# jhbastek/PhysicsInformedDiffusionModels

Hardware: NVIDIA H100
Metric: train samples/s Darcy 64x64 PIDM (higher is better)
Workload: dtype bf16

## Files before the change

### include/pidm.h

```cpp
#ifndef PIDM_H_
#define PIDM_H_

#ifdef __cplusplus
extern "C" {
#endif

#ifndef PIDM_F32
#define PIDM_F32 0
#define PIDM_BF16 1
#endif

const char* pidm_last_error(void);
int pidm_version(void);

int pidm_qsample(const float* x0, const float* noise, const long long* t, const float* sqrt_ab,
                 const float* sqrt_1mab, float* xt, int B, int per_sample, void* stream);
int pidm_posterior_step(const float* x_t, const float* x0_pred, const float* z, float* out, float coef1, float coef2,
                        float sigma, long long n, void* stream);
int pidm_axpby_per_sample(const float* a, const float* x, const float* b, const float* y, const float* c,
                          const float* z, float* out, int B, int per_sample, void* stream);
int pidm_ddim_coefs(const long long* t, const long long* t_next, const float* posterior_mean_coef1,
                    const float* posterior_mean_coef2, const float* sqrt_recip_alphas, const float* noise_mean_coeff,
                    const float* alphas_prod, float* coef_x0, float* coef_x, int B, void* stream);
int pidm_scale(const float* x, const float* alpha_dev, float* out, long long n, void* stream);

int pidm_toy_pidm_loss(const float* target, const float* output, const float* residual, const float* ineq,
                       const float* opt, const long long* t, const float* p2_loss_weight,
                       const float* posterior_var_clipped, float c_data, float c_residual, float c_ineq, float lambda_opt,
                       float* sums7, float* grad_output, float* grad_residual, float* grad_ineq, float* grad_opt, int B,
                       int D, void* stream);

#define PIDM_DARCY_PIXELS_AT_BOUNDARY 1
#define PIDM_DARCY_PERIODIC 2
int pidm_darcy_residual_fwd(const float* x0hat, const float* f_s, float* residual, int B, int pixels,
                            float domain_length, int reverse_d1, int flags, void* stream);
int pidm_darcy_residual_bwd(const float* x0hat, const float* f_s, const float* grad_residual, float* grad_x0hat, int B,
                            int pixels, float domain_length, int reverse_d1, int flags, void* stream);
#define PIDM_FD_PERIODIC 8
int pidm_fd_stencil(const float* u, float* out, int planes, int pixels, int mode, float d0, float d1, void* stream);
int pidm_darcy_pidm_loss(const float* x0hat, const float* model_out, const float* target, const float* f_s,
                         const long long* t, const float* p2_loss_weight, const float* posterior_var_clipped,
                         float c_data, float c_residual, float* sums3, float* grad_x0hat, float* grad_model_out, int B,
                         int pixels, float domain_length, int reverse_d1, int flags, void* stream);
int pidm_darcy_jacobian_max(const float* x0hat, float* max_dr_dp, int B, int pixels, float domain_length, int reverse_d1,
                            int flags, void* stream);

int pidm_nchw_to_nhwc(const float* src, void* dst, int B, int C, int HW, int Cpad, int dtype, void* stream);
int pidm_nhwc_to_nchw(const void* src, float* dst, int B, int C, int HW, int Cpad, int dtype, void* stream);
int pidm_add(const void* a, const void* b, void* out, long long n, int dtype, void* stream);
int pidm_gelu_fwd(const void* x, void* y, long long n, int dtype, void* stream);
int pidm_gelu_bwd(const void* x, const void* dy, void* dx, long long n, int dtype, void* stream);
int pidm_concat_channels(const void* a, const void* b, void* out, long long rows, int Ca, int Cb, int dtype, void* stream);
int pidm_split_channels(const void* g, void* ga, void* gb, long long rows, int Ca, int Cb, int dtype, void* stream);

int pidm_pack_entry_size(void);
int pidm_pack_weights(const void* table_dev, int n_entries, int dtype, void* stream);
int pidm_pack_pair_entry_size(void);
int pidm_pack_weights_pairs(const void* table_dev, const int* tile_map_dev, int tile_base, int n_tiles, int max_taps,
                            int dtype, void* stream);
int pidm_conv2d_simt(const void* x, const void* w_packed, const float* bias, const void* residual, void* y, int B,
                     int H, int W, int Cin, int Ho, int Wo, int Cout, int KH, int KW, int stride, int pad,
                     int transposed, int dtype, void* stream);
int pidm_conv2d_wgrad_simt(const void* x, const void* dy, float* dw, float* dbias, int B, int H, int W, int Cin,
                           int Cin_real, int Ho, int Wo, int Cout, int KH, int KW, int stride, int pad, int transposed,
                           long long w_stride_n, long long w_stride_c, int dtype, void* stream);
int pidm_debug_set_trace(void* buf);
int pidm_conv2d_tc_general(const void* x, const void* w_packed, const float* bias, const void* residual, void* y, int B,
                           int H, int W, int Cin, int Ho, int Wo, int Cout, int KH, int KW, int stride, int pad,
                           int transposed, float* gn_sums, int gn_groups, int gn_sums_zeroed, void* stream);
int pidm_conv2d_tc_general_supported(int B, int H, int W, int Cin, int Ho, int Wo, int Cout, int KH, int KW, int stride,
                                     int pad, int transposed);
int pidm_conv2d_tc_plan(int B, int H, int W, int Cin, int Ho, int Wo, int Cout, int KH, int KW, int stride, int pad,
                        int transposed, int* out);
int pidm_conv2d_wgrad_tc(const void* a, const void* b, float* dw, int B, int HA, int WA, int CA, int CA_real, int GH,
                         int GW, int CB, int KH, int KW, int a_stride, int pad, long long s_row, long long s_col,
                         void* stream);
int pidm_conv2d_wgrad_tc_supported(int B, int GH, int GW, int CA, int CB, int KH, int KW, int a_stride);
int pidm_conv2d_wgrad_tc_plan(int B, int HA, int WA, int CA, int CA_real, int GH, int GW, int CB, int KH, int KW,
                              int a_stride, int pad, long long s_row, long long s_col, int* out);
int pidm_colsum(const void* x, float* out, long long M, int C, int dtype, void* stream);

int pidm_groupnorm_silu_fwd(const void* x, const float* gamma, const float* beta, const float* scale_shift,
                            const void* residual, void* y, float* sums, int stats_precomputed, int B, int HW, int C, int G,
                            float eps, int dtype, void* stream);
int pidm_groupnorm_silu_bwd(const void* x, const void* dy, const float* sums, const float* gamma, const float* beta,
                            const float* scale_shift, void* dx, float* dgamma, float* dbeta, float* d_scale_shift,
                            float* dbias_of_producer, float* workspace, int B, int HW, int C, int G, float eps,
                            int dtype, void* stream);
int pidm_layernorm_c_fwd(const void* x, const float* gamma, void* y, long long M, int C, float eps, int dtype, void* stream);
int pidm_layernorm_c_bwd(const void* x, const void* dy, const float* gamma, void* dx, float* dgamma,
                         const void* dx_residual , long long M, int C,
                         float eps, int dtype, void* stream);

int pidm_linattn_fused_supported(int C, int heads, int N, int dtype);
int pidm_linattn_fused_workspace_floats(int B, int N);
int pidm_linattn_fused_plan(int B, int N, int* out);
int pidm_linattn_fused_fwd(const void* xn, const void* w_qkv, void* out, float* ctx, float* kmax, float* kzinv,
                           float* workspace, int B, int N, void* stream);
int pidm_linattn_fused_bwd(const void* xn, const void* w_qkv, const void* dout, const float* ctx, const float* kmax,
                           const float* kzinv, void* dxn, float* dctx, int B, int N, void* stream);
int pidm_linattn_fused_wgrad(const void* xn, const void* w_qkv, const void* dout, const float* ctx, const float* dctx,
                             const float* kmax, const float* kzinv, float* grad_w, int B, int N, long long w_stride_n,
                             long long w_stride_c, void* stream);
int pidm_linattn_workspace_floats(int B, int N, int heads);
int pidm_linattn_fwd(const void* qkv, void* out, float* ctx, float* kmax, float* kzinv, float* workspace, int B, int N,
                     int heads, int dtype, void* stream);
int pidm_linattn_bwd(const void* qkv, const void* dout, const float* ctx, const float* kmax, const float* kzinv,
                     void* dqkv, float* dctx_scratch, int B, int N, int heads, int dtype, void* stream);
int pidm_attn_fwd(const void* qkv, void* out, int B, int n_tokens, int heads, int dtype, void* stream);
int pidm_attn_bwd(const void* qkv, const void* dout, void* dqkv, int B, int n_tokens, int heads, int dtype, void* stream);

int pidm_time_embed_fwd(const long long* t, const float* W1, const float* b1, const float* W2, const float* b2,
                        float* emb, float* h1, float* temb, float* silu_t, int B, int dim, int td, void* stream);
int pidm_time_embed_bwd(const float* d_silu_t, const float* emb, const float* h1, const float* temb, const float* W2,
                        float* dW1, float* db1, float* dW2, float* db2, float* workspace, int B, int dim, int td,
                        int parts, void* stream);
int pidm_mlp_entry_size(void);
int pidm_block_mlps_fwd(const void* table_dev, int n_entries, int max_rows, const float* silu_t, int B, int td,
                        void* stream);
int pidm_block_mlps_bwd(const void* table_dev, int n_entries, int max_rows, const float* silu_t, float* d_silu_t, int B,
                        int td, int parts, void* stream);

int pidm_head_fwd(const void* x, const float* w, const float* bias, float* y, int B, int HW, int C, int O,
                  int sigmoid_last, int dtype, void* stream);
int pidm_head_bwd(const void* x, const float* w, const float* y, const float* dy, void* dx, float* dw, float* db, int B,
                  int HW, int C, int O, int sigmoid_last, int dtype, void* stream);

int pidm_sumsq(const float* x, long long n, float* out, float* workspace, void* stream);
int pidm_adam_ema_step(float* param, float* grad, float* exp_avg, float* exp_avg_sq, float* ema_shadow, long long n,
                       float lr, double beta1, double beta2, float eps, int step, int* step_counter_dev,
                       const float* grad_norm_sq_dev, float grad_scale, float max_norm, float ema_mu,
                       int ema_first_step, int zero_grad, void* stream);

int pidm_mechanics_residual_fwd(const float* u, const float* rho, const float* bcs, const float* KE, float* residual,
                                float* compliance, int B, int nel, void* stream);
int pidm_mechanics_residual_bwd(const float* u, const float* rho, const float* bcs, const float* KE,
                                const float* grad_residual, const float* grad_compliance, float* grad_u, float* grad_rho,
                                float* workspace , int B, int nel, void* stream);
int pidm_mech_pidm_loss(const float* u, const float* rho, const float* x0, const float* residual, const float* compliance,
                        const float* vf, const long long* t, const float* p2_loss_weight,
                        const float* posterior_var_clipped, float c_data, float c_residual, float c_ineq,
                        float lambda_opt, float* sums6, float* grad_u, float* grad_rho, float* grad_residual,
                        float* grad_compliance, int B, int nel, void* stream);
int pidm_bilinear_resize_fwd(const float* x, float* y, int planes, int in, int out, void* stream);
int pidm_bilinear_resize_bwd(const float* dy, float* dx, int planes, int in, int out, void* stream);

#ifdef __cplusplus
}
#endif
#endif
```

### physicsinformeddiffusionmodels_b200/_lib.py

```python
import ctypes
import os

import torch

_HERE = os.path.dirname(os.path.abspath(__file__))
LIB_PATH = os.path.join(_HERE, 'libpidm.so')

P = ctypes.c_void_p
I = ctypes.c_int
L = ctypes.c_longlong
F = ctypes.c_float
D = ctypes.c_double

_SIGS = {
    'pidm_qsample': [P, P, P, P, P, P, I, I, P],
    'pidm_posterior_step': [P, P, P, P, F, F, F, L, P],
    'pidm_scale': [P, P, P, L, P],
    'pidm_ddim_coefs': [P, P, P, P, P, P, P, P, P, I, P],
    'pidm_axpby_per_sample': [P, P, P, P, P, P, P, I, I, P],
    'pidm_toy_pidm_loss': [P, P, P, P, P, P, P, P, F, F, F, F, P, P, P, P, P, I, I, P],
    'pidm_fd_stencil': [P, P, I, I, I, F, F, P],
    'pidm_darcy_residual_fwd': [P, P, P, I, I, F, I, I, P],
    'pidm_darcy_residual_bwd': [P, P, P, P, I, I, F, I, I, P],
    'pidm_darcy_jacobian_max': [P, P, I, I, F, I, I, P],
    'pidm_darcy_pidm_loss': [P, P, P, P, P, P, P, F, F, P, P, P, I, I, F, I, I, P],
    'pidm_nchw_to_nhwc': [P, P, I, I, I, I, I, P],
    'pidm_nhwc_to_nchw': [P, P, I, I, I, I, I, P],
    'pidm_add': [P, P, P, L, I, P],
    'pidm_gelu_fwd': [P, P, L, I, P],
    'pidm_gelu_bwd': [P, P, P, L, I, P],
    'pidm_concat_channels': [P, P, P, L, I, I, I, P],
    'pidm_split_channels': [P, P, P, L, I, I, I, P],
    'pidm_pack_entry_size': [],
    'pidm_pack_weights': [P, I, I, P],
    'pidm_pack_pair_entry_size': [],
    'pidm_pack_weights_pairs': [P, P, I, I, I, I, P],
    'pidm_conv2d_simt': [P, P, P, P, P, I, I, I, I, I, I, I, I, I, I, I, I, I, P],
    'pidm_conv2d_wgrad_simt': [P, P, P, P, I, I, I, I, I, I, I, I, I, I, I, I, I, L, L, I, P],
    'pidm_debug_set_trace': [P],
    'pidm_conv2d_tc_general': [P, P, P, P, P, I, I, I, I, I, I, I, I, I, I, I, I, P, I, I, P],
    'pidm_conv2d_tc_general_supported': [I, I, I, I, I, I, I, I, I, I, I, I],
    'pidm_conv2d_tc_plan': [I, I, I, I, I, I, I, I, I, I, I, I, P],
    'pidm_conv2d_wgrad_tc': [P, P, P, I, I, I, I, I, I, I, I, I, I, I, I, L, L, P],
    'pidm_conv2d_wgrad_tc_supported': [I, I, I, I, I, I, I, I],
    'pidm_conv2d_wgrad_tc_plan': [I, I, I, I, I, I, I, I, I, I, I, I, L, L, P],
    'pidm_colsum': [P, P, L, I, I, P],
    'pidm_groupnorm_silu_fwd': [P, P, P, P, P, P, P, I, I, I, I, I, F, I, P],
    'pidm_groupnorm_silu_bwd': [P, P, P, P, P, P, P, P, P, P, P, P, I, I, I, I, F, I, P],
    'pidm_layernorm_c_fwd': [P, P, P, L, I, F, I, P],
    'pidm_layernorm_c_bwd': [P, P, P, P, P, P, L, I, F, I, P],
    'pidm_linattn_workspace_floats': [I, I, I],
    'pidm_linattn_fused_supported': [I, I, I, I],
    'pidm_linattn_fused_workspace_floats': [I, I],
    'pidm_linattn_fused_plan': [I, I, P],
    'pidm_linattn_fused_fwd': [P, P, P, P, P, P, P, I, I, P],
    'pidm_linattn_fused_bwd': [P, P, P, P, P, P, P, P, I, I, P],
    'pidm_linattn_fused_wgrad': [P, P, P, P, P, P, P, P, I, I, L, L, P],
    'pidm_linattn_fwd': [P, P, P, P, P, P, I, I, I, I, P],
    'pidm_linattn_bwd': [P, P, P, P, P, P, P, I, I, I, I, P],
    'pidm_attn_fwd': [P, P, I, I, I, I, P],
    'pidm_attn_bwd': [P, P, P, I, I, I, I, P],
    'pidm_time_embed_fwd': [P, P, P, P, P, P, P, P, P, I, I, I, P],
    'pidm_time_embed_bwd': [P, P, P, P, P, P, P, P, P, P, I, I, I, I, P],
    'pidm_mlp_entry_size': [],
    'pidm_block_mlps_fwd': [P, I, I, P, I, I, P],
    'pidm_block_mlps_bwd': [P, I, I, P, P, I, I, I, P],
    'pidm_head_fwd': [P, P, P, P, I, I, I, I, I, I, P],
    'pidm_head_bwd': [P, P, P, P, P, P, P, I, I, I, I, I, I, P],
    'pidm_sumsq': [P, L, P, P, P],
    'pidm_adam_ema_step': [P, P, P, P, P, L, F, D, D, F, I, P, P, F, F, F, I, I, P],
    'pidm_mechanics_residual_fwd': [P, P, P, P, P, P, I, I, P],
    'pidm_mechanics_residual_bwd': [P, P, P, P, P, P, P, P, P, I, I, P],
    'pidm_mech_pidm_loss': [P, P, P, P, P, P, P, P, P, F, F, F, F, P, P, P, P, P, I, I, P],
    'pidm_bilinear_resize_fwd': [P, P, I, I, I, P],
    'pidm_bilinear_resize_bwd': [P, P, I, I, I, P],
    'pidm_version': [],
}
_VALUE_RETURN = {'pidm_pack_entry_size', 'pidm_pack_pair_entry_size', 'pidm_mlp_entry_size', 'pidm_linattn_workspace_floats', 'pidm_version',
                 'pidm_linattn_fused_supported', 'pidm_linattn_fused_workspace_floats',
                 'pidm_conv2d_tc_supported', 'pidm_conv2d_wgrad_tc_supported', 'pidm_conv2d_tc_general_supported',
                 'pidm_conv2d_tc_plan', 'pidm_conv2d_wgrad_tc_plan', 'pidm_linattn_fused_plan'}

if not os.path.exists(LIB_PATH):
    raise ImportError(f'{LIB_PATH} is missing: build it with `python __graft_entry__.py` (nvcc, sm_90a). '
                      'There is no CPU / PyTorch fallback for the PIDM hot path.')

_lib = ctypes.CDLL(LIB_PATH)
_lib.pidm_last_error.restype = ctypes.c_char_p
_lib.pidm_last_error.argtypes = []
for _n, _a in _SIGS.items():
    _f = getattr(_lib, _n)
    _f.argtypes = _a
    _f.restype = ctypes.c_int

launch_count = 0


def exported_symbols():
    return sorted(_SIGS) + ['pidm_last_error']


def ptr(t):
    if t is None:
        return None
    return t.data_ptr()


def stream():
    return torch.cuda.current_stream().cuda_stream


def call(name, *args):
    global launch_count
    conv = []
    for a in args:
        if isinstance(a, torch.Tensor):
            conv.append(a.data_ptr())
        else:
            conv.append(a)
    rc = getattr(_lib, name)(*conv)
    if name in _VALUE_RETURN:
        return rc
    launch_count += 1
    if rc != 0:
        raise RuntimeError(f'{name} failed (code {rc}): {_lib.pidm_last_error().decode()}')
    return 0


DTYPE_CODE = {torch.float32: 0, torch.bfloat16: 1}
```

### physicsinformeddiffusionmodels_b200/csrc/attention_fused.cu

```cuda
#define PIDM_PDL_GROUP 1
#include "common.cuh"
#include "mma_util.cuh"
#include "pidm.h"

namespace pidm {

constexpr int LF_C = 32;

__device__ __forceinline__ uint32_t movm_t(uint32_t x) {
    uint32_t y;
    asm volatile("movmatrix.sync.aligned.m8n8.trans.b16 %0, %1;" : "=r"(y) : "r"(x));
    return y;
}

__device__ __forceinline__ void load_w_frags(uint32_t (&w)[2][4][2], const __nv_bfloat16* __restrict__ Wrows, int lane) {
    const int g = lane >> 2, t = lane & 3;
#pragma unroll
    for (int ks = 0; ks < 2; ++ks)
#pragma unroll
        for (int nt = 0; nt < 4; ++nt) {
            const uint32_t* row = reinterpret_cast<const uint32_t*>(Wrows + (size_t)(nt * 8 + g) * LF_C + ks * 16 + 2 * t);
            w[ks][nt][0] = __ldg(row);
            w[ks][nt][1] = __ldg(row + 4);
        }
}
template <int MT>
__device__ __forceinline__ void load_x_frags(uint32_t (&a)[MT][2][4], const __nv_bfloat16* Xs, int lane) {
#pragma unroll
    for (int mt = 0; mt < MT; ++mt)
#pragma unroll
        for (int ks = 0; ks < 2; ++ks) frag_a_rowmajor(a[mt][ks], Xs, LW_PITCH, mt * 16, ks * 16, lane);
}
template <int MT>
__device__ __forceinline__ void project(float (&c)[MT][4][4], const uint32_t (&a)[MT][2][4], const uint32_t (&w)[2][4][2]) {
#pragma unroll
    for (int mt = 0; mt < MT; ++mt)
#pragma unroll
        for (int nt = 0; nt < 4; ++nt) {
#pragma unroll
            for (int i = 0; i < 4; ++i) c[mt][nt][i] = 0.f;
#pragma unroll
            for (int ks = 0; ks < 2; ++ks) mma_bf16(c[mt][nt], a[mt][ks], w[ks][nt][0], w[ks][nt][1]);
        }
}
__device__ __forceinline__ void frag_softmax(float (&c)[4][4], float mul) {
#pragma unroll
    for (int half = 0; half < 2; ++half) {
        float mx = -INFINITY;
#pragma unroll
        for (int nt = 0; nt < 4; ++nt) mx = fmaxf(mx, fmaxf(c[nt][half * 2], c[nt][half * 2 + 1]));
        mx = fmaxf(mx, __shfl_xor_sync(0xffffffffu, mx, 1));
        mx = fmaxf(mx, __shfl_xor_sync(0xffffffffu, mx, 2));
        float s = 0.f;
#pragma unroll
        for (int nt = 0; nt < 4; ++nt) {
            c[nt][half * 2] = __expf(c[nt][half * 2] - mx);
            c[nt][half * 2 + 1] = __expf(c[nt][half * 2 + 1] - mx);
            s += c[nt][half * 2] + c[nt][half * 2 + 1];
        }
        s += __shfl_xor_sync(0xffffffffu, s, 1);
        s += __shfl_xor_sync(0xffffffffu, s, 2);
        const float inv = mul / s;
#pragma unroll
        for (int nt = 0; nt < 4; ++nt) { c[nt][half * 2] *= inv; c[nt][half * 2 + 1] *= inv; }
    }
}
__device__ __forceinline__ void c_to_a(uint32_t (&a)[2][4], const float (&c)[4][4]) {
#pragma unroll
    for (int ks = 0; ks < 2; ++ks) {
        a[ks][0] = pack_bf16(c[2 * ks][0], c[2 * ks][1]);
        a[ks][1] = pack_bf16(c[2 * ks][2], c[2 * ks][3]);
        a[ks][2] = pack_bf16(c[2 * ks + 1][0], c[2 * ks + 1][1]);
        a[ks][3] = pack_bf16(c[2 * ks + 1][2], c[2 * ks + 1][3]);
    }
}
__device__ __forceinline__ void load_cols(float (&v)[8], const float* __restrict__ src, int lane) {
    const int t = lane & 3;
#pragma unroll
    for (int nt = 0; nt < 4; ++nt) { v[nt * 2] = src[nt * 8 + 2 * t]; v[nt * 2 + 1] = src[nt * 8 + 2 * t + 1]; }
}

constexpr int LFS_STAGES = 2;
__global__ void __launch_bounds__(256) laf_kmax_kernel(const __nv_bfloat16* __restrict__ xn,
                                                       const __nv_bfloat16* __restrict__ W, float* __restrict__ part,
                                                       int N, int rows_per_chunk) {
    pdl_trigger();
    pdl_wait();
    extern __shared__ __align__(16) unsigned char raw[];
    const int b = blockIdx.y, chunk = blockIdx.x, lane = threadIdx.x & 31, h = threadIdx.x >> 5;
    __nv_bfloat16* ring = reinterpret_cast<__nv_bfloat16*>(raw) + (size_t)h * (LFS_STAGES * LW_TILE);
    const int n_begin = chunk * rows_per_chunk, n_end = min(N, n_begin + rows_per_chunk);
    const int n_tiles = (n_end - n_begin) / 32;
    const __nv_bfloat16* xsrc = xn + ((size_t)b * N + n_begin) * LF_C;
    auto issue = [&](int it) {
        if (it < n_tiles) lw_issue<32>(ring + (size_t)(it % LFS_STAGES) * LW_TILE, xsrc + (size_t)it * 32 * LF_C, LF_C, lane);
        cp_commit();
    };
#pragma unroll
    for (int s = 0; s < LFS_STAGES; ++s) issue(s);
    uint32_t wk[2][4][2];
    load_w_frags(wk, W + (size_t)(LM_HID + h * LM_D) * LF_C, lane);
    float m[8];
#pragma unroll
    for (int i = 0; i < 8; ++i) m[i] = -INFINITY;
    for (int it = 0; it < n_tiles; ++it) {
        cp_wait<LFS_STAGES - 1>();
        __syncwarp();
        uint32_t ax[2][2][4];
        load_x_frags<2>(ax, ring + (size_t)(it % LFS_STAGES) * LW_TILE, lane);
        __syncwarp();
        issue(it + LFS_STAGES);
        float ck[2][4][4];
        project<2>(ck, ax, wk);
#pragma unroll
        for (int nt = 0; nt < 4; ++nt)
#pragma unroll
            for (int j = 0; j < 2; ++j)
                m[nt * 2 + j] = fmaxf(fmaxf(m[nt * 2 + j], fmaxf(ck[0][nt][j], ck[0][nt][2 + j])),
                                      fmaxf(ck[1][nt][j], ck[1][nt][2 + j]));
    }
#pragma unroll
    for (int off = 4; off < 32; off <<= 1)
#pragma unroll
        for (int i = 0; i < 8; ++i) m[i] = fmaxf(m[i], __shfl_xor_sync(0xffffffffu, m[i], off));
    if (lane < 4) {
        float* o = part + ((size_t)b * gridDim.x + chunk) * LM_HID + h * LM_D;
#pragma unroll
        for (int nt = 0; nt < 4; ++nt)
#pragma unroll
            for (int j = 0; j < 2; ++j) o[nt * 8 + 2 * lane + j] = m[nt * 2 + j];
    }
}

__global__ void laf_finalize_kernel(float* __restrict__ ctx, float* __restrict__ kzinv, int n_rows) {
    pdl_trigger();
    pdl_wait();
    const int row = blockIdx.x * (blockDim.x / 32) + (threadIdx.x >> 5), lane = threadIdx.x & 31;
    if (row >= n_rows) return;
    const float zi = 1.f / kzinv[row];
    ctx[(size_t)row * LM_D + lane] *= zi;
    __syncwarp();
    if (lane == 0) kzinv[row] = zi;
}

template <int MODE>
struct LfcCfg {
    static constexpr int STAGES = MODE == 0 ? 4 : 2;
    static constexpr int STAGE_ELEMS = MODE == 0 ? LW_TILE : 2 * LW_TILE;
    static constexpr size_t SMEM = (size_t)LM_HEADS * STAGES * STAGE_ELEMS * 2 + (size_t)LM_HEADS * 2 * LM_D * 4;
};
template <int MODE>
__global__ void __launch_bounds__(256, 2) laf_ctx_kernel(const __nv_bfloat16* __restrict__ xn, const __nv_bfloat16* __restrict__ W,
                                                      const __nv_bfloat16* __restrict__ dout, const float* __restrict__ part,
                                                      int n_stat_chunks, float* __restrict__ kmax, float* __restrict__ kzinv,
                                                      float* __restrict__ ctx, int N, int chunk_px, float scale) {
    pdl_trigger();
    pdl_wait();
    extern __shared__ __align__(16) unsigned char raw[];
    constexpr int LFC_STAGES = LfcCfg<MODE>::STAGES, LFC_STAGE_ELEMS = LfcCfg<MODE>::STAGE_ELEMS;
    const int b = blockIdx.y, chunk = blockIdx.x, lane = threadIdx.x & 31, h = threadIdx.x >> 5;
    __nv_bfloat16* ring = reinterpret_cast<__nv_bfloat16*>(raw) + (size_t)h * (LFC_STAGES * LFC_STAGE_ELEMS);
    float* sM = reinterpret_cast<float*>(raw + (size_t)LM_HEADS * LFC_STAGES * LFC_STAGE_ELEMS * 2) + h * 2 * LM_D;
    float* sZi = sM + LM_D;
    const int n_begin = chunk * chunk_px, n_end = min(N, n_begin + chunk_px);
    const int n_tiles = (n_end - n_begin) / 32;
    const size_t pix0 = (size_t)b * N + n_begin;
    const __nv_bfloat16* xsrc = xn + pix0 * LF_C;
    const __nv_bfloat16* gsrc = (MODE == 1) ? dout + pix0 * LM_HID + h * LM_D : nullptr;
    auto issue = [&](int it) {
        if (it < n_tiles) {
            __nv_bfloat16* buf = ring + (size_t)(it % LFC_STAGES) * LFC_STAGE_ELEMS;
            lw_issue<32>(buf, xsrc + (size_t)it * 32 * LF_C, LF_C, lane);
            if (MODE == 1) lw_issue<32>(buf + LW_TILE, gsrc + (size_t)it * 32 * LM_HID, LM_HID, lane);
        }
        cp_commit();
    };
#pragma unroll
    for (int s = 0; s < LFC_STAGES; ++s) issue(s);
    uint32_t w0[2][4][2], w1[2][4][2];
    load_w_frags(w0, W + (size_t)((MODE == 0 ? LM_HID : 0) + h * LM_D) * LF_C, lane);
    if (MODE == 0) load_w_frags(w1, W + (size_t)(2 * LM_HID + h * LM_D) * LF_C, lane);
    float Mc[8];
    float zacc[8];
#pragma unroll
    for (int i = 0; i < 8; ++i) zacc[i] = 0.f;
    if (MODE == 0) {
        const int c = h * LM_D + lane;
        float M = -INFINITY;
        for (int i = 0; i < n_stat_chunks; ++i) M = fmaxf(M, part[((size_t)b * n_stat_chunks + i) * LM_HID + c]);
        sM[lane] = M;
        if (chunk == 0) kmax[(size_t)b * LM_HID + c] = M;
        __syncwarp();
        load_cols(Mc, sM, lane);
    }
    float acc[2][4][4];
#pragma unroll
    for (int i = 0; i < 2; ++i)
#pragma unroll
        for (int j = 0; j < 4; ++j)
#pragma unroll
            for (int k = 0; k < 4; ++k) acc[i][j][k] = 0.f;
    for (int it = 0; it < n_tiles; ++it) {
        cp_wait<LFC_STAGES - 1>();
        __syncwarp();
        const __nv_bfloat16* buf = ring + (size_t)(it % LFC_STAGES) * LFC_STAGE_ELEMS;
        uint32_t ax[2][2][4];
        load_x_frags<2>(ax, buf, lane);
        uint32_t bv[2][4][2];
        if (MODE == 1) {
#pragma unroll
            for (int ks = 0; ks < 2; ++ks) {
                uint32_t b01[4], b23[4];
                frag_b_krows(b01, buf + LW_TILE, LW_PITCH, ks * 16, 0, lane);
                frag_b_krows(b23, buf + LW_TILE, LW_PITCH, ks * 16, 16, lane);
                bv[ks][0][0] = b01[0]; bv[ks][0][1] = b01[1]; bv[ks][1][0] = b01[2]; bv[ks][1][1] = b01[3];
                bv[ks][2][0] = b23[0]; bv[ks][2][1] = b23[1]; bv[ks][3][0] = b23[2]; bv[ks][3][1] = b23[3];
            }
        }
        __syncwarp();
        issue(it + LFC_STAGES);
        float cw[2][4][4];
        project<2>(cw, ax, w0);
        if (MODE == 0) {
#pragma unroll
            for (int mt = 0; mt < 2; ++mt)
#pragma unroll
                for (int nt = 0; nt < 4; ++nt)
#pragma unroll
                    for (int i = 0; i < 4; ++i) {
                        cw[mt][nt][i] = __expf(cw[mt][nt][i] - Mc[nt * 2 + (i & 1)]);
                        zacc[nt * 2 + (i & 1)] += cw[mt][nt][i];
                    }
            float cv[2][4][4];
            project<2>(cv, ax, w1);
#pragma unroll
            for (int mt = 0; mt < 2; ++mt)
#pragma unroll
                for (int nt = 0; nt < 4; ++nt) {
                    bv[mt][nt][0] = movm_t(pack_bf16(cv[mt][nt][0], cv[mt][nt][1]));
                    bv[mt][nt][1] = movm_t(pack_bf16(cv[mt][nt][2], cv[mt][nt][3]));
                }
        } else {
            frag_softmax(cw[0], scale);
            frag_softmax(cw[1], scale);
        }
#pragma unroll
        for (int mt = 0; mt < 2; ++mt) {
#pragma unroll
            for (int md = 0; md < 2; ++md) {
                uint32_t a[4];
                a[0] = movm_t(pack_bf16(cw[mt][2 * md][0], cw[mt][2 * md][1]));
                a[1] = movm_t(pack_bf16(cw[mt][2 * md + 1][0], cw[mt][2 * md + 1][1]));
                a[2] = movm_t(pack_bf16(cw[mt][2 * md][2], cw[mt][2 * md][3]));
                a[3] = movm_t(pack_bf16(cw[mt][2 * md + 1][2], cw[mt][2 * md + 1][3]));
#pragma unroll
                for (int ne = 0; ne < 4; ++ne) mma_bf16(acc[md][ne], a, bv[mt][ne][0], bv[mt][ne][1]);
            }
        }
    }
    const int g = lane >> 2, t = lane & 3;
    if (MODE == 0) {
#pragma unroll
        for (int off = 4; off < 32; off <<= 1)
#pragma unroll
            for (int i = 0; i < 8; ++i) zacc[i] += __shfl_xor_sync(0xffffffffu, zacc[i], off);
        if (lane < 4) {
#pragma unroll
            for (int nt = 0; nt < 4; ++nt)
#pragma unroll
                for (int j = 0; j < 2; ++j)
                    atomicAdd(kzinv + (size_t)b * LM_HID + h * LM_D + nt * 8 + 2 * lane + j, zacc[nt * 2 + j]);
        }
    }
    float* cb = ctx + ((size_t)b * LM_HEADS + h) * LM_D * LM_D;
#pragma unroll
    for (int md = 0; md < 2; ++md)
#pragma unroll
        for (int half = 0; half < 2; ++half) {
            const int d = md * 16 + g + half * 8;
            const float f = (MODE == 0) ? 1.f / (float)N : 1.f;
#pragma unroll
            for (int ne = 0; ne < 4; ++ne) {
                const int e = ne * 8 + 2 * t;
                atomicAdd(cb + d * LM_D + e, acc[md][ne][half * 2] * f);
                atomicAdd(cb + d * LM_D + e + 1, acc[md][ne][half * 2 + 1] * f);
            }
        }
}

constexpr int LFO_STAGES = 2;
__global__ void __launch_bounds__(256) laf_out_kernel(const __nv_bfloat16* __restrict__ xn, const __nv_bfloat16* __restrict__ W,
                                                      const float* __restrict__ ctx, __nv_bfloat16* __restrict__ out, int N,
                                                      int chunk_px, float scale) {
    pdl_trigger();
    pdl_wait();
    extern __shared__ __align__(16) unsigned char raw[];
    const int b = blockIdx.y, chunk = blockIdx.x, lane = threadIdx.x & 31, h = threadIdx.x >> 5;
    __nv_bfloat16* ring = reinterpret_cast<__nv_bfloat16*>(raw) + (size_t)h * ((LFO_STAGES + 1) * LW_TILE);
    __nv_bfloat16* Os = ring + LFO_STAGES * LW_TILE;
    const int n_begin = chunk * chunk_px, n_end = min(N, n_begin + chunk_px);
    const int n_tiles = (n_end - n_begin) / 32;
    const size_t pix0 = (size_t)b * N + n_begin;
    const __nv_bfloat16* xsrc = xn + pix0 * LF_C;
    __nv_bfloat16* odst = out + pix0 * LM_HID + h * LM_D;
    auto issue = [&](int it) {
        if (it < n_tiles) lw_issue<32>(ring + (size_t)(it % LFO_STAGES) * LW_TILE, xsrc + (size_t)it * 32 * LF_C, LF_C, lane);
        cp_commit();
    };
#pragma unroll
    for (int s = 0; s < LFO_STAGES; ++s) issue(s);
    uint32_t wq[2][4][2];
    load_w_frags(wq, W + (size_t)(h * LM_D) * LF_C, lane);
    const float* ch = ctx + ((size_t)b * LM_HEADS + h) * LM_D * LM_D;
    uint32_t bf[2][4][2];
#pragma unroll
    for (int ks = 0; ks < 2; ++ks)
#pragma unroll
        for (int nt = 0; nt < 4; ++nt) frag_b_global<true>(bf[ks][nt], ch, ks * 16, nt * 8, lane);
    const int g = lane >> 2, t = lane & 3;
    for (int it = 0; it < n_tiles; ++it) {
        cp_wait<LFO_STAGES - 1>();
        __syncwarp();
        uint32_t ax[2][2][4];
        load_x_frags<2>(ax, ring + (size_t)(it % LFO_STAGES) * LW_TILE, lane);
        __syncwarp();
        issue(it + LFO_STAGES);
        float cq[2][4][4];
        project<2>(cq, ax, wq);
#pragma unroll
        for (int mt = 0; mt < 2; ++mt) {
            frag_softmax(cq[mt], scale);
            uint32_t a[2][4];
            c_to_a(a, cq[mt]);
            float c[4][4];
#pragma unroll
            for (int i = 0; i < 4; ++i)
#pragma unroll
                for (int k = 0; k < 4; ++k) c[i][k] = 0.f;
#pragma unroll
            for (int ks = 0; ks < 2; ++ks)
#pragma unroll
                for (int nt = 0; nt < 4; ++nt) mma_bf16(c[nt], a[ks], bf[ks][nt][0], bf[ks][nt][1]);
#pragma unroll
            for (int nt = 0; nt < 4; ++nt) {
                __nv_bfloat16* o = Os + (size_t)(mt * 16 + g) * LW_PITCH + nt * 8 + 2 * t;
                *reinterpret_cast<uint32_t*>(o) = pack_bf16(c[nt][0], c[nt][1]);
                *reinterpret_cast<uint32_t*>(o + 8 * LW_PITCH) = pack_bf16(c[nt][2], c[nt][3]);
            }
        }
        __syncwarp();
        lw_store<32>(odst + (size_t)it * 32 * LM_HID, LM_HID, Os, lane);
        __syncwarp();
    }
}

constexpr int LFB_ROWS = 16;
constexpr int LFB_STAGES = 4;
constexpr int LFB_TILE = LFB_ROWS * LW_PITCH;

struct LfbTile {
    uint32_t ax[1][2][4], ag[2][4];
};
__device__ __forceinline__ void lfb_dq(float (&dq)[4][4], const LfbTile& tl, const uint32_t (&wq)[2][4][2],
                                       const uint32_t (&bc)[2][4][2], float scale) {
    float c1[1][4][4], c2[4][4];
    project<1>(c1, tl.ax, wq);
    frag_softmax(c1[0], 1.f);
#pragma unroll
    for (int nt = 0; nt < 4; ++nt) {
#pragma unroll
        for (int i = 0; i < 4; ++i) c2[nt][i] = 0.f;
#pragma unroll
        for (int ks = 0; ks < 2; ++ks) mma_bf16(c2[nt], tl.ag[ks], bc[ks][nt][0], bc[ks][nt][1]);
    }
#pragma unroll
    for (int half = 0; half < 2; ++half) {
        float dot = 0.f;
#pragma unroll
        for (int nt = 0; nt < 4; ++nt)
            dot += c1[0][nt][half * 2] * c2[nt][half * 2] + c1[0][nt][half * 2 + 1] * c2[nt][half * 2 + 1];
        dot += __shfl_xor_sync(0xffffffffu, dot, 1);
        dot += __shfl_xor_sync(0xffffffffu, dot, 2);
#pragma unroll
        for (int nt = 0; nt < 4; ++nt)
#pragma unroll
            for (int j = 0; j < 2; ++j) dq[nt][half * 2 + j] = scale * c1[0][nt][half * 2 + j] * (c2[nt][half * 2 + j] - dot);
    }
}
__device__ __forceinline__ void lfb_dkdv(float (&dk)[4][4], float (&dv)[4][4], const uint32_t (&ax)[1][2][4],
                                         const uint32_t (&wk)[2][4][2], const uint32_t (&wv)[2][4][2],
                                         const uint32_t (&bd)[2][4][2], const uint32_t (&bt)[2][4][2],
                                         const float (&Mc)[8], const float (&Zc)[8], const float (&cdc)[8], float invN) {
    float c1[1][4][4];
    uint32_t a[2][4];
    project<1>(c1, ax, wv);
    c_to_a(a, c1[0]);
#pragma unroll
    for (int nt = 0; nt < 4; ++nt) {
#pragma unroll
        for (int i = 0; i < 4; ++i) dk[nt][i] = 0.f;
#pragma unroll
        for (int ks = 0; ks < 2; ++ks) mma_bf16(dk[nt], a[ks], bd[ks][nt][0], bd[ks][nt][1]);
    }
    project<1>(c1, ax, wk);
#pragma unroll
    for (int nt = 0; nt < 4; ++nt)
#pragma unroll
        for (int i = 0; i < 4; ++i) {
            c1[0][nt][i] = __expf(c1[0][nt][i] - Mc[nt * 2 + (i & 1)]) * Zc[nt * 2 + (i & 1)];
            dk[nt][i] = c1[0][nt][i] * (dk[nt][i] * invN - cdc[nt * 2 + (i & 1)]);
        }
    c_to_a(a, c1[0]);
#pragma unroll
    for (int nt = 0; nt < 4; ++nt) {
#pragma unroll
        for (int i = 0; i < 4; ++i) dv[nt][i] = 0.f;
#pragma unroll
        for (int ks = 0; ks < 2; ++ks) mma_bf16(dv[nt], a[ks], bt[ks][nt][0], bt[ks][nt][1]);
#pragma unroll
        for (int i = 0; i < 4; ++i) dv[nt][i] *= invN;
    }
}
__device__ __forceinline__ void lfb_cd(float (&cdc)[8], float* scd, const float* __restrict__ cg, const float* __restrict__ dg,
                                       int lane) {
    float s = 0.f;
#pragma unroll
    for (int e = 0; e < LM_D; e += 4) {
        const float4 x = *reinterpret_cast<const float4*>(dg + lane * LM_D + e);
        const float4 y = *reinterpret_cast<const float4*>(cg + lane * LM_D + e);
        s += x.x * y.x + x.y * y.y + x.z * y.z + x.w * y.w;
    }
    scd[lane] = s;
    __syncwarp();
    load_cols(cdc, scd, lane);
}

constexpr int LFB_STAGE_ELEMS = (1 + LM_HEADS) * LFB_TILE;
constexpr int LFB_W_PITCH = LF_C + 8;
constexpr int LFB_R_PITCH = LF_C + 8;
constexpr size_t LAF_BWD_SMEM = (size_t)LFB_STAGES * LFB_STAGE_ELEMS * 2 + (size_t)3 * LM_HID * LFB_W_PITCH * 2 +
                                (size_t)LM_HEADS * LFB_ROWS * LFB_R_PITCH * 4 + (size_t)LM_HEADS * LM_D * 4;

__device__ __forceinline__ void mma_w(float (&c)[4][4], const uint32_t (&g)[2][4], const __nv_bfloat16* Wh, int lane) {
#pragma unroll
    for (int kd = 0; kd < 2; ++kd)
#pragma unroll
        for (int np = 0; np < 2; ++np) {
            uint32_t bw[4];
            frag_b_krows(bw, Wh, LFB_W_PITCH, kd * 16, np * 16, lane);
            mma_bf16(c[2 * np], g[kd], bw[0], bw[1]);
            mma_bf16(c[2 * np + 1], g[kd], bw[2], bw[3]);
        }
}

__global__ void __launch_bounds__(256) laf_bwd_kernel(const __nv_bfloat16* __restrict__ xn, const __nv_bfloat16* __restrict__ W,
                                                      const __nv_bfloat16* __restrict__ dout, const float* __restrict__ ctx,
                                                      const float* __restrict__ dctx, const float* __restrict__ kmax,
                                                      const float* __restrict__ kzinv, __nv_bfloat16* __restrict__ dxn,
                                                      int N, int chunk_px, float scale) {
    pdl_trigger();
    pdl_wait();
    extern __shared__ __align__(16) unsigned char raw[];
    const int b = blockIdx.y, chunk = blockIdx.x, lane = threadIdx.x & 31, h = threadIdx.x >> 5;
    __nv_bfloat16* ring = reinterpret_cast<__nv_bfloat16*>(raw);
    __nv_bfloat16* Ws = ring + LFB_STAGES * LFB_STAGE_ELEMS;
    float* R = reinterpret_cast<float*>(Ws + 3 * LM_HID * LFB_W_PITCH);
    float* scd = R + LM_HEADS * LFB_ROWS * LFB_R_PITCH + h * LM_D;
    const int n_begin = chunk * chunk_px, n_end = min(N, n_begin + chunk_px);
    const int n_tiles = (n_end - n_begin) / LFB_ROWS;
    const size_t pix0 = (size_t)b * N + n_begin;
    const __nv_bfloat16* xsrc = xn + pix0 * LF_C;
    const __nv_bfloat16* gsrc = dout + pix0 * LM_HID + h * LM_D;
    for (int i = threadIdx.x; i < 3 * LM_HID * (LF_C / 8); i += blockDim.x)
        cp_async16(Ws + (i >> 2) * LFB_W_PITCH + (i & 3) * 8, W + (size_t)(i >> 2) * LF_C + (i & 3) * 8);
    cp_commit();
    auto issue = [&](int it) {
        if (it < n_tiles) {
            __nv_bfloat16* buf = ring + (size_t)(it % LFB_STAGES) * LFB_STAGE_ELEMS;
            if (h == 0) lw_issue<LFB_ROWS>(buf, xsrc + (size_t)it * LFB_ROWS * LF_C, LF_C, lane);
            lw_issue<LFB_ROWS>(buf + (1 + h) * LFB_TILE, gsrc + (size_t)it * LFB_ROWS * LM_HID, LM_HID, lane);
        }
        cp_commit();
    };
#pragma unroll
    for (int s = 0; s < LFB_STAGES - 1; ++s) issue(s);
    const float* cg = ctx + ((size_t)b * LM_HEADS + h) * LM_D * LM_D;
    const float* dg = dctx + ((size_t)b * LM_HEADS + h) * LM_D * LM_D;
    float Mc[8], Zc[8], cdc[8];
    lfb_cd(cdc, scd, cg, dg, lane);
    load_cols(Mc, kmax + (size_t)b * LM_HID + h * LM_D, lane);
    load_cols(Zc, kzinv + (size_t)b * LM_HID + h * LM_D, lane);
    uint32_t wq[2][4][2], wk[2][4][2], wv[2][4][2];
    load_w_frags(wq, W + (size_t)(h * LM_D) * LF_C, lane);
    load_w_frags(wk, W + (size_t)(LM_HID + h * LM_D) * LF_C, lane);
    load_w_frags(wv, W + (size_t)(2 * LM_HID + h * LM_D) * LF_C, lane);
    uint32_t bc[2][4][2], bd[2][4][2], bt[2][4][2];
#pragma unroll
    for (int ks = 0; ks < 2; ++ks)
#pragma unroll
        for (int nt = 0; nt < 4; ++nt) {
            frag_b_global<false>(bc[ks][nt], cg, ks * 16, nt * 8, lane);
            frag_b_global<false>(bd[ks][nt], dg, ks * 16, nt * 8, lane);
            frag_b_global<true>(bt[ks][nt], dg, ks * 16, nt * 8, lane);
        }
    const int g = lane >> 2, t = lane & 3;
    const float invN = 1.f / (float)N;
    const __nv_bfloat16* Wq = Ws + (size_t)(h * LM_D) * LFB_W_PITCH;
    const __nv_bfloat16* Wk = Wq + (size_t)LM_HID * LFB_W_PITCH;
    const __nv_bfloat16* Wv = Wk + (size_t)LM_HID * LFB_W_PITCH;
    float* Rw = R + h * LFB_ROWS * LFB_R_PITCH;
    const int rrow = threadIdx.x >> 4, rcol = (threadIdx.x & 15) * 2;
    for (int it = 0; it < n_tiles; ++it) {
        cp_wait<LFB_STAGES - 2>();
        __syncthreads();
        issue(it + LFB_STAGES - 1);
        const __nv_bfloat16* buf = ring + (size_t)(it % LFB_STAGES) * LFB_STAGE_ELEMS;
        LfbTile tl;
        load_x_frags<1>(tl.ax, buf, lane);
        frag_a_rowmajor(tl.ag[0], buf + (1 + h) * LFB_TILE, LW_PITCH, 0, 0, lane);
        frag_a_rowmajor(tl.ag[1], buf + (1 + h) * LFB_TILE, LW_PITCH, 0, 16, lane);
        float dx[4][4];
#pragma unroll
        for (int nt = 0; nt < 4; ++nt)
#pragma unroll
            for (int i = 0; i < 4; ++i) dx[nt][i] = 0.f;
        uint32_t a[2][4];
        {
            float dq[4][4];
            lfb_dq(dq, tl, wq, bc, scale);
            c_to_a(a, dq);
            mma_w(dx, a, Wq, lane);
        }
        {
            float dk[4][4], dv[4][4];
            lfb_dkdv(dk, dv, tl.ax, wk, wv, bd, bt, Mc, Zc, cdc, invN);
            c_to_a(a, dk);
            mma_w(dx, a, Wk, lane);
            c_to_a(a, dv);
            mma_w(dx, a, Wv, lane);
        }
#pragma unroll
        for (int nt = 0; nt < 4; ++nt)
#pragma unroll
            for (int half = 0; half < 2; ++half)
                *reinterpret_cast<float2*>(Rw + (g + half * 8) * LFB_R_PITCH + nt * 8 + 2 * t) =
                    make_float2(dx[nt][half * 2], dx[nt][half * 2 + 1]);
        __syncthreads();
        float sx = 0.f, sy = 0.f;
#pragma unroll
        for (int w = 0; w < LM_HEADS; ++w) {
            const float2 v = *reinterpret_cast<const float2*>(R + (w * LFB_ROWS + rrow) * LFB_R_PITCH + rcol);
            sx += v.x;
            sy += v.y;
        }
        *reinterpret_cast<uint32_t*>(dxn + (pix0 + (size_t)it * LFB_ROWS + rrow) * LF_C + rcol) = pack_bf16(sx, sy);
    }
}

template <int PART>
struct LfwCfg {
    static constexpr int MATS = PART == 0 ? 1 : 2;
    static constexpr int STAGE_ELEMS = (PART == 0 ? 2 : 1) * LFB_TILE;
    static constexpr int S_PITCH = LM_D + 1;
    static_assert(LFB_STAGES * STAGE_ELEMS * 2 >= LM_D * S_PITCH * 4, "the epilogue staging reuses the tile ring");
    static constexpr size_t SMEM = (size_t)LM_HEADS * (LFB_STAGES * STAGE_ELEMS * 2 + LM_D * 4);
};

__device__ __forceinline__ void acc_gtx(float (&acc)[2][4][4], const float (&gf)[4][4], const uint32_t (&bx)[2][4]) {
#pragma unroll
    for (int md = 0; md < 2; ++md) {
        uint32_t a[4];
        a[0] = movm_t(pack_bf16(gf[2 * md][0], gf[2 * md][1]));
        a[1] = movm_t(pack_bf16(gf[2 * md + 1][0], gf[2 * md + 1][1]));
        a[2] = movm_t(pack_bf16(gf[2 * md][2], gf[2 * md][3]));
        a[3] = movm_t(pack_bf16(gf[2 * md + 1][2], gf[2 * md + 1][3]));
#pragma unroll
        for (int np = 0; np < 2; ++np) {
            mma_bf16(acc[md][2 * np], a, bx[np][0], bx[np][1]);
            mma_bf16(acc[md][2 * np + 1], a, bx[np][2], bx[np][3]);
        }
    }
}

template <int PART>
__global__ void __launch_bounds__(256) laf_wgrad_kernel(const __nv_bfloat16* __restrict__ xn, const __nv_bfloat16* __restrict__ W,
                                                        const __nv_bfloat16* __restrict__ dout, const float* __restrict__ ctx,
                                                        const float* __restrict__ dctx, const float* __restrict__ kmax,
                                                        const float* __restrict__ kzinv, float* __restrict__ grad_w, int N,
                                                        int chunk_px, long long w_stride_n, long long w_stride_c, float scale) {
    pdl_trigger();
    pdl_wait();
    extern __shared__ __align__(16) unsigned char raw[];
    constexpr int MATS = LfwCfg<PART>::MATS, STAGE_ELEMS = LfwCfg<PART>::STAGE_ELEMS, S_PITCH = LfwCfg<PART>::S_PITCH;
    const int b = blockIdx.y, chunk = blockIdx.x, lane = threadIdx.x & 31, h = threadIdx.x >> 5;
    __nv_bfloat16* ring = reinterpret_cast<__nv_bfloat16*>(raw) + (size_t)h * (LFB_STAGES * STAGE_ELEMS);
    float* scd = reinterpret_cast<float*>(raw + (size_t)LM_HEADS * LFB_STAGES * STAGE_ELEMS * 2) + h * LM_D;
    const int n_begin = chunk * chunk_px, n_end = min(N, n_begin + chunk_px);
    const int n_tiles = (n_end - n_begin) / LFB_ROWS;
    const size_t pix0 = (size_t)b * N + n_begin;
    const __nv_bfloat16* xsrc = xn + pix0 * LF_C;
    const __nv_bfloat16* gsrc = dout + pix0 * LM_HID + h * LM_D;
    auto issue = [&](int it) {
        if (it < n_tiles) {
            __nv_bfloat16* buf = ring + (size_t)(it % LFB_STAGES) * STAGE_ELEMS;
            lw_issue<LFB_ROWS>(buf, xsrc + (size_t)it * LFB_ROWS * LF_C, LF_C, lane);
            if (PART == 0) lw_issue<LFB_ROWS>(buf + LFB_TILE, gsrc + (size_t)it * LFB_ROWS * LM_HID, LM_HID, lane);
        }
        cp_commit();
    };
#pragma unroll
    for (int s = 0; s < LFB_STAGES; ++s) issue(s);
    const float* cg = ctx + ((size_t)b * LM_HEADS + h) * LM_D * LM_D;
    const float* dg = dctx + ((size_t)b * LM_HEADS + h) * LM_D * LM_D;
    float Mc[8], Zc[8], cdc[8];
    uint32_t w0[2][4][2], w1[2][4][2];
    uint32_t b0[2][4][2], b1[2][4][2];
    if (PART == 0) {
        load_w_frags(w0, W + (size_t)(h * LM_D) * LF_C, lane);
    } else {
        lfb_cd(cdc, scd, cg, dg, lane);
        load_cols(Mc, kmax + (size_t)b * LM_HID + h * LM_D, lane);
        load_cols(Zc, kzinv + (size_t)b * LM_HID + h * LM_D, lane);
        load_w_frags(w0, W + (size_t)(LM_HID + h * LM_D) * LF_C, lane);
        load_w_frags(w1, W + (size_t)(2 * LM_HID + h * LM_D) * LF_C, lane);
    }
#pragma unroll
    for (int ks = 0; ks < 2; ++ks)
#pragma unroll
        for (int nt = 0; nt < 4; ++nt) {
            frag_b_global<false>(b0[ks][nt], PART == 0 ? cg : dg, ks * 16, nt * 8, lane);
            if (PART == 1) frag_b_global<true>(b1[ks][nt], dg, ks * 16, nt * 8, lane);
        }
    const float invN = 1.f / (float)N;
    float acc[MATS][2][4][4];
#pragma unroll
    for (int m = 0; m < MATS; ++m)
#pragma unroll
        for (int i = 0; i < 2; ++i)
#pragma unroll
            for (int j = 0; j < 4; ++j)
#pragma unroll
                for (int k = 0; k < 4; ++k) acc[m][i][j][k] = 0.f;
    for (int it = 0; it < n_tiles; ++it) {
        cp_wait<LFB_STAGES - 1>();
        __syncwarp();
        const __nv_bfloat16* buf = ring + (size_t)(it % LFB_STAGES) * STAGE_ELEMS;
        LfbTile tl;
        load_x_frags<1>(tl.ax, buf, lane);
        uint32_t bx[2][4];
        frag_b_krows(bx[0], buf, LW_PITCH, 0, 0, lane);
        frag_b_krows(bx[1], buf, LW_PITCH, 0, 16, lane);
        if (PART == 0) {
            frag_a_rowmajor(tl.ag[0], buf + LFB_TILE, LW_PITCH, 0, 0, lane);
            frag_a_rowmajor(tl.ag[1], buf + LFB_TILE, LW_PITCH, 0, 16, lane);
        }
        __syncwarp();
        issue(it + LFB_STAGES);
        if (PART == 0) {
            float dq[4][4];
            lfb_dq(dq, tl, w0, b0, scale);
            acc_gtx(acc[0], dq, bx);
        } else {
            float dk[4][4], dv[4][4];
            lfb_dkdv(dk, dv, tl.ax, w0, w1, b0, b1, Mc, Zc, cdc, invN);
            acc_gtx(acc[0], dk, bx);
            acc_gtx(acc[MATS - 1], dv, bx);
        }
    }
    cp_wait<0>();
    __syncwarp();
    float* S = reinterpret_cast<float*>(ring);
    const int g = lane >> 2, t = lane & 3;
#pragma unroll
    for (int m = 0; m < MATS; ++m) {
#pragma unroll
        for (int md = 0; md < 2; ++md)
#pragma unroll
            for (int nc = 0; nc < 4; ++nc)
#pragma unroll
                for (int i = 0; i < 4; ++i) S[(md * 16 + g + 8 * (i >> 1)) * S_PITCH + nc * 8 + 2 * t + (i & 1)] = acc[m][md][nc][i];
        __syncwarp();
        float* dst = grad_w + (long long)((PART + m) * LM_HID + h * LM_D) * w_stride_n + lane * w_stride_c;
#pragma unroll 4
        for (int d = 0; d < LM_D; ++d) atomicAdd(dst + d * w_stride_n, S[d * S_PITCH + lane]);
        __syncwarp();
    }
}

constexpr size_t LAF_STATS_SMEM = (size_t)LM_HEADS * LFS_STAGES * LW_TILE * 2;
constexpr size_t LAF_OUT_SMEM = (size_t)LM_HEADS * (LFO_STAGES + 1) * LW_TILE * 2;

static int laf_attrs() {
    static bool done = false;
    if (!done) {
        PIDM_CUDA(cudaFuncSetAttribute(laf_kmax_kernel, cudaFuncAttributeMaxDynamicSharedMemorySize, (int)LAF_STATS_SMEM));
        PIDM_CUDA(cudaFuncSetAttribute(laf_ctx_kernel<0>, cudaFuncAttributeMaxDynamicSharedMemorySize, (int)LfcCfg<0>::SMEM));
        PIDM_CUDA(cudaFuncSetAttribute(laf_ctx_kernel<1>, cudaFuncAttributeMaxDynamicSharedMemorySize, (int)LfcCfg<1>::SMEM));
        PIDM_CUDA(cudaFuncSetAttribute(laf_out_kernel, cudaFuncAttributeMaxDynamicSharedMemorySize, (int)LAF_OUT_SMEM));
        PIDM_CUDA(cudaFuncSetAttribute(laf_bwd_kernel, cudaFuncAttributeMaxDynamicSharedMemorySize, (int)LAF_BWD_SMEM));
        PIDM_CUDA(cudaFuncSetAttribute(laf_wgrad_kernel<0>, cudaFuncAttributeMaxDynamicSharedMemorySize, (int)LfwCfg<0>::SMEM));
        PIDM_CUDA(cudaFuncSetAttribute(laf_wgrad_kernel<1>, cudaFuncAttributeMaxDynamicSharedMemorySize, (int)LfwCfg<1>::SMEM));
        done = true;
    }
    return 0;
}

static int laf_chunk_px(int B, int N, int ctas_per_sm) {
    int k = (num_sms() * ctas_per_sm) / B;
    if (k < 1) k = 1;
    int px = ((N + k - 1) / k + 31) / 32 * 32;
    if (px < 64) px = 64;
    if (px > N) px = N;
    return px;
}
static int laf_stat_chunks(int N) {
    int c = N / 128;
    if (c < 1) c = 1;
    if (c > 16) c = 16;
    return c;
}

}
using namespace pidm;

extern "C" int pidm_linattn_fused_supported(int C, int heads, int N, int dtype) {
    return (C == LF_C && heads == LM_HEADS && dtype == PIDM_BF16 && N % 128 == 0) ? 1 : 0;
}

extern "C" int pidm_linattn_fused_workspace_floats(int B, int N) { return B * laf_stat_chunks(N) * LM_HID; }

extern "C" int pidm_linattn_fused_plan(int B, int N, int* out) {
    PIDM_REQUIRE(N % 128 == 0 && B > 0, "linattn_fused_plan: N must be a multiple of 128 (got %d)", N);
    const int v[5] = {laf_stat_chunks(N), laf_chunk_px(B, N, 2), laf_chunk_px(B, N, 3), laf_chunk_px(B, N, 1),
                      laf_chunk_px(B, N, 1)};
    for (int i = 0; i < 5; ++i) out[i] = v[i];
    return 0;
}

extern "C" int pidm_linattn_fused_fwd(const void* xn, const void* w_qkv, void* out, float* ctx, float* kmax, float* kzinv,
                                      float* workspace, int B, int N, void* stream) {
    PIDM_REQUIRE(N % 128 == 0, "linattn_fused: N must be a multiple of 128 (got %d)", N);
    cudaStream_t st = (cudaStream_t)stream;
    if (int e = laf_attrs()) return e;
    const float scale = 0.17677669529663687f;
    const __nv_bfloat16* x = (const __nv_bfloat16*)xn;
    const __nv_bfloat16* w = (const __nv_bfloat16*)w_qkv;
    PIDM_CUDA(cudaMemsetAsync(ctx, 0, (size_t)B * LM_HEADS * LM_D * LM_D * sizeof(float), st));
    PIDM_CUDA(cudaMemsetAsync(kzinv, 0, (size_t)B * LM_HID * sizeof(float), st));
    const int chunks = laf_stat_chunks(N);
    const int rpc = N / chunks;
    PIDM_REQUIRE(rpc % 32 == 0 && rpc * chunks == N, "linattn_fused: bad statistics chunking for N=%d", N);
    PIDM_CUDA(launch_pdl(laf_kmax_kernel, dim3(dim3(chunks, B)), dim3(256), (size_t)(LAF_STATS_SMEM), st, x, w, workspace, N, rpc));
    const int cpx = laf_chunk_px(B, N, 2);
    PIDM_CUDA(launch_pdl(laf_ctx_kernel<0>, dim3(dim3((N + cpx - 1) / cpx, B)), dim3(256), (size_t)(LfcCfg<0>::SMEM), st, x, w, nullptr, workspace, chunks, kmax, kzinv,
                                                                             ctx, N, cpx, scale));
    PIDM_CUDA(launch_pdl(laf_finalize_kernel, dim3((B * LM_HID + 7) / 8), dim3(256), (size_t)(0), st, ctx, kzinv, B * LM_HID));
    const int opx = laf_chunk_px(B, N, 3);
    PIDM_CUDA(launch_pdl(laf_out_kernel, dim3(dim3((N + opx - 1) / opx, B)), dim3(256), (size_t)(LAF_OUT_SMEM), st, x, w, ctx, (__nv_bfloat16*)out, N, opx, scale));
    PIDM_LAUNCH_CHECK("linattn_fused_fwd");
    return 0;
}

extern "C" int pidm_linattn_fused_bwd(const void* xn, const void* w_qkv, const void* dout, const float* ctx,
                                      const float* kmax, const float* kzinv, void* dxn, float* dctx, int B, int N,
                                      void* stream) {
    PIDM_REQUIRE(N % 128 == 0, "linattn_fused: N must be a multiple of 128 (got %d)", N);
    cudaStream_t st = (cudaStream_t)stream;
    if (int e = laf_attrs()) return e;
    const float scale = 0.17677669529663687f;
    const __nv_bfloat16* x = (const __nv_bfloat16*)xn;
    const __nv_bfloat16* w = (const __nv_bfloat16*)w_qkv;
    PIDM_CUDA(cudaMemsetAsync(dctx, 0, (size_t)B * LM_HEADS * LM_D * LM_D * sizeof(float), st));
    const int cpx = laf_chunk_px(B, N, 2);
    PIDM_CUDA(launch_pdl(laf_ctx_kernel<1>, dim3(dim3((N + cpx - 1) / cpx, B)), dim3(256), (size_t)(LfcCfg<1>::SMEM), st, x, w, (const __nv_bfloat16*)dout, nullptr, 0,
                                                                             nullptr, nullptr, dctx, N, cpx, scale));
    const int bpx = laf_chunk_px(B, N, 1);
    PIDM_CUDA(launch_pdl(laf_bwd_kernel, dim3(dim3((N + bpx - 1) / bpx, B)), dim3(256), (size_t)(LAF_BWD_SMEM), st, x, w, (const __nv_bfloat16*)dout, ctx, dctx, kmax,
                                                                          kzinv, (__nv_bfloat16*)dxn, N, bpx, scale));
    PIDM_LAUNCH_CHECK("linattn_fused_bwd");
    return 0;
}

extern "C" int pidm_linattn_fused_wgrad(const void* xn, const void* w_qkv, const void* dout, const float* ctx,
                                        const float* dctx, const float* kmax, const float* kzinv, float* grad_w, int B,
                                        int N, long long w_stride_n, long long w_stride_c, void* stream) {
    PIDM_REQUIRE(N % 128 == 0, "linattn_fused: N must be a multiple of 128 (got %d)", N);
    cudaStream_t st = (cudaStream_t)stream;
    if (int e = laf_attrs()) return e;
    const float scale = 0.17677669529663687f;
    const __nv_bfloat16* x = (const __nv_bfloat16*)xn;
    const __nv_bfloat16* w = (const __nv_bfloat16*)w_qkv;
    const __nv_bfloat16* g = (const __nv_bfloat16*)dout;
    const int px = laf_chunk_px(B, N, 1);
    const dim3 grid((N + px - 1) / px, B);
    PIDM_CUDA(launch_pdl(laf_wgrad_kernel<0>, grid, dim3(256), LfwCfg<0>::SMEM, st, x, w, g, ctx, dctx, kmax, kzinv, grad_w, N,
                         px, w_stride_n, w_stride_c, scale));
    PIDM_CUDA(launch_pdl(laf_wgrad_kernel<1>, grid, dim3(256), LfwCfg<1>::SMEM, st, x, w, g, ctx, dctx, kmax, kzinv, grad_w, N,
                         px, w_stride_n, w_stride_c, scale));
    PIDM_LAUNCH_CHECK("linattn_fused_wgrad");
    return 0;
}
```

### physicsinformeddiffusionmodels_b200/ops.py

```python
import os

import torch

from . import _lib
from ._lib import call, stream

_TC_HARD_OFF = os.environ.get('PIDM_DISABLE_TC') == '1'
_STATE = {'act_dtype': torch.bfloat16, 'use_tc': not _TC_HARD_OFF}


def set_precision(name):
    _STATE['act_dtype'] = {'bf16': torch.bfloat16, 'fp32': torch.float32}[name]


def set_tensor_core_conv(flag):
    _STATE['use_tc'] = bool(flag) and not _TC_HARD_OFF


def act_dtype():
    return _STATE['act_dtype']


def _code(t):
    return _lib.DTYPE_CODE[t.dtype]


def _grad_buffer(p):
    g = getattr(p, '_pidm_grad', None)
    if g is not None:
        return g, None
    z = torch.zeros_like(p)
    return z, z


def _need_cuda(*ts):
    for t in ts:
        if t is not None and not t.is_cuda:
            raise RuntimeError('physicsinformeddiffusionmodels_b200 runs on CUDA (H100) only: got a CPU tensor. '
                               'There is no CPU fallback on the product path.')


def _need_f32(**named):
    for k, t in named.items():
        if t is None:
            continue
        if not t.is_cuda:
            raise RuntimeError(f'{k}: expected a CUDA tensor (no CPU fallback on the product path)')
        if t.dtype != torch.float32 or not t.is_contiguous():
            raise RuntimeError(f'{k}: expected a contiguous float32 tensor, got {t.dtype}, strides {t.stride()}')


def nchw_to_nhwc(x, cpad, dtype=None):
    _need_cuda(x)
    B, C, H, W = x.shape
    dtype = dtype or act_dtype()
    y = torch.empty(B, H, W, cpad, device=x.device, dtype=dtype)
    call('pidm_nchw_to_nhwc', x.contiguous().float(), y, B, C, H * W, cpad, _lib.DTYPE_CODE[dtype], stream())
    return y


def nhwc_to_nchw(x, C=None):
    B, H, W, Cp = x.shape
    C = C or Cp
    y = torch.empty(B, C, H, W, device=x.device, dtype=torch.float32)
    call('pidm_nhwc_to_nchw', x, y, B, C, H * W, Cp, _code(x), stream())
    return y


class _Add(torch.autograd.Function):
    @staticmethod
    def forward(ctx, a, b):
        o = torch.empty_like(a)
        call('pidm_add', a, b, o, a.numel(), _code(a), stream())
        return o

    @staticmethod
    def backward(ctx, g):
        return g, g


def add(a, b):
    return _Add.apply(a.contiguous(), b.contiguous())


class _Gelu(torch.autograd.Function):
    @staticmethod
    def forward(ctx, x):
        y = torch.empty_like(x)
        call('pidm_gelu_fwd', x, y, x.numel(), _code(x), stream())
        ctx.save_for_backward(x)
        return y

    @staticmethod
    def backward(ctx, dy):
        (x,) = ctx.saved_tensors
        dx = torch.empty_like(x)
        call('pidm_gelu_bwd', x, dy.contiguous(), dx, x.numel(), _code(x), stream())
        return dx


def gelu(x):
    return _Gelu.apply(x.contiguous())


class _Stash(torch.autograd.Function):

    @staticmethod
    def forward(ctx, x, link):
        ctx.link = link
        link['expect_skip'] = True
        return x.view_as(x)

    @staticmethod
    def backward(ctx, g):
        ctx.link['skip'] = g.contiguous()
        return None, None


def stash_grad(x, link):
    return _Stash.apply(x, link)


def _take_skip(link):
    if link is None or not link.get('expect_skip'):
        return None
    if 'skip' not in link:
        raise RuntimeError('skip-connection gradient was expected but has not been produced yet (autograd order)')
    return link.pop('skip')


class _Concat(torch.autograd.Function):
    @staticmethod
    def forward(ctx, a, b):
        B, H, W, Ca = a.shape
        Cb = b.shape[-1]
        o = torch.empty(B, H, W, Ca + Cb, device=a.device, dtype=a.dtype)
        call('pidm_concat_channels', a, b, o, B * H * W, Ca, Cb, _code(a), stream())
        ctx.shapes = (a.shape, b.shape)
        return o

    @staticmethod
    def backward(ctx, g):
        sa, sb = ctx.shapes
        g = g.contiguous()
        ga = torch.empty(sa, device=g.device, dtype=g.dtype)
        gb = torch.empty(sb, device=g.device, dtype=g.dtype)
        call('pidm_split_channels', g, ga, gb, sa[0] * sa[1] * sa[2], sa[3], sb[3], _code(g), stream())
        return ga, gb


def concat(a, b):
    return _Concat.apply(a.contiguous(), b.contiguous())


_ZERO_POOL = {'buf': None, 'cur': 0}


def zero_pool_begin(nfloats, device):
    _ZERO_POOL['buf'] = torch.zeros(int(nfloats), device=device, dtype=torch.float32)
    _ZERO_POOL['cur'] = 0


def zero_pool_end():
    _ZERO_POOL['buf'] = None


def _zero_take(*shape):
    buf = _ZERO_POOL['buf']
    n = 1
    for d in shape:
        n *= int(d)
    n_al = (n + 31) // 32 * 32
    if buf is None or _ZERO_POOL['cur'] + n_al > buf.numel():
        return None
    out = buf[_ZERO_POOL['cur']:_ZERO_POOL['cur'] + n].view(*shape)
    _ZERO_POOL['cur'] += n_al
    return out


def _conv_launch(x, wp, bias, residual, y, g, transposed, gn_sums=None, gn_groups=0, gn_zeroed=False):
    B, H, W, Cin, Ho, Wo, Cout, KH, KW, stride, pad = g
    tr = 1 if transposed else 0
    if (_STATE['use_tc'] and x.dtype == torch.bfloat16
            and call('pidm_conv2d_tc_general_supported', B, H, W, Cin, Ho, Wo, Cout, KH, KW, stride, pad, tr)):
        cpg = Cout // gn_groups if gn_groups else 0
        fuse = gn_sums is not None and (cpg in (4, 8, 16) or (cpg > 0 and cpg % 32 == 0))
        call('pidm_conv2d_tc_general', x, wp, bias, residual, y, B, H, W, Cin, Ho, Wo, Cout, KH, KW, stride, pad, tr,
             gn_sums if fuse else None, gn_groups if fuse else 0, 1 if gn_zeroed else 0, stream())
        return fuse
    else:
        call('pidm_conv2d_simt', x, wp, bias, residual, y, B, H, W, Cin, Ho, Wo, Cout, KH, KW, stride, pad,
             1 if transposed else 0, _code(x), stream())
        return False


class _Conv2d(torch.autograd.Function):

    @staticmethod
    def forward(ctx, x, weight, bias, residual, spec, link, skip):
        B, H, W, Cin = x.shape
        Ho, Wo = spec.out_hw(H, W)
        y = torch.empty(B, Ho, Wo, spec.cout, device=x.device, dtype=x.dtype)
        g = (B, H, W, Cin, Ho, Wo, spec.cout, spec.kh, spec.kw, spec.stride, spec.pad)
        sums, zeroed = None, False
        if link is not None:
            sums = _zero_take(B, link['groups'], 2)
            zeroed = sums is not None
            if sums is None:
                sums = torch.empty(B, link['groups'], 2, device=x.device, dtype=torch.float32)
        fused = _conv_launch(x, spec.wp_fwd, bias, residual, y, g, spec.transposed, sums, link['groups'] if link else 0,
                             zeroed)
        if link is not None:
            link['sums'] = sums if fused else None
            link['bias'] = bias
        ctx.save_for_backward(x, weight, bias)
        ctx.spec, ctx.g, ctx.has_res, ctx.link, ctx.skip = spec, g, residual is not None, link, skip
        if skip is not None and skip[0] == 'park':
            skip[1]['expect_skip'] = True
        return y

    @staticmethod
    def backward(ctx, dy):
        x, weight, bias = ctx.saved_tensors
        dy = dy.contiguous()
        skip = ctx.skip
        dgrad_res = _take_skip(skip[1]) if (skip is not None and skip[0] == 'take' and ctx.needs_input_grad[0]) else None
        dx, gw_ret, gb_ret = _conv_backward(x, weight, bias, ctx.spec, ctx.g, dy, ctx.needs_input_grad[0], ctx.link,
                                            dgrad_res)
        if skip is not None and skip[0] == 'park':
            skip[1]['skip'] = dx
            dx = None
        return dx, gw_ret, gb_ret, (dy if ctx.has_res else None), None, None, None


_SIDE = {'streams': [], 'next': 0, 'keep': [], 'active': False}
_N_SIDE = max(1, int(os.environ.get('PIDM_SIDE_STREAMS', '1')))


def side_stream_begin():
    if os.environ.get('PIDM_NO_SIDE_STREAM') == '1':
        return
    while len(_SIDE['streams']) < _N_SIDE:
        _SIDE['streams'].append(torch.cuda.Stream())
    _SIDE['active'] = True
    _SIDE['next'] = 0
    _SIDE['keep'] = []


def side_stream_join():
    if _SIDE['active']:
        for st in _SIDE['streams']:
            torch.cuda.current_stream().wait_stream(st)
        _SIDE['keep'] = []
        _SIDE['active'] = False


_FORK = {'stream': None}


def fork_stream():
    if _FORK['stream'] is None:
        _FORK['stream'] = torch.cuda.Stream()
    _FORK['stream'].wait_stream(torch.cuda.current_stream())
    return _FORK['stream']


def _wgrad_stream(*operands):
    if not _SIDE['active']:
        return stream()
    side = _SIDE['streams'][_SIDE['next']]
    _SIDE['next'] = (_SIDE['next'] + 1) % len(_SIDE['streams'])
    side.wait_stream(torch.cuda.current_stream())
    _SIDE['keep'].extend(operands)
    return side.cuda_stream


def _conv_backward(x, weight, bias, spec, g, dy, need_dx, link=None, dgrad_residual=None):
    B, H, W, Cin, Ho, Wo, Cout, KH, KW, stride, pad = g
    dx = None
    if need_dx or dgrad_residual is not None:
        dx = torch.empty_like(x)
        if stride == 1 and not spec.transposed:
            gd = (B, Ho, Wo, Cout, H, W, Cin, KH, KW, 1, KH - 1 - pad)
            _conv_launch(dy, spec.wp_dgrad, None, dgrad_residual, dx, gd, False)
        else:
            gd = (B, Ho, Wo, Cout, H, W, Cin, KH, KW, stride, pad)
            _conv_launch(dy, spec.wp_dgrad, None, dgrad_residual, dx, gd, not spec.transposed)
    gw_buf, gw_ret = _grad_buffer(weight)
    gb_buf, gb_ret = (None, None) if bias is None else _grad_buffer(bias)
    if link is not None and 'dbias' in link:
        gb_buf, gb_ret = None, link.pop('dbias')
    use_tc = _STATE['use_tc'] and x.dtype == torch.bfloat16
    ws = _wgrad_stream(x, dy)
    if use_tc and not spec.transposed and call('pidm_conv2d_wgrad_tc_supported', B, Ho, Wo, Cin, Cout, KH, KW, stride):
        call('pidm_conv2d_wgrad_tc', x, dy, gw_buf, B, H, W, Cin, spec.cin_real, Ho, Wo, Cout, KH, KW, stride, pad,
             spec.w_stride_c, spec.w_stride_n, ws)
        if gb_buf is not None:
            call('pidm_colsum', dy, gb_buf, B * Ho * Wo, Cout, _code(dy), ws)
    elif use_tc and spec.transposed and call('pidm_conv2d_wgrad_tc_supported', B, H, W, Cout, Cin, KH, KW, stride):
        call('pidm_conv2d_wgrad_tc', dy, x, gw_buf, B, Ho, Wo, Cout, Cout, H, W, Cin, KH, KW, stride, pad,
             spec.w_stride_n, spec.w_stride_c, ws)
        if gb_buf is not None:
            call('pidm_colsum', dy, gb_buf, B * Ho * Wo, Cout, _code(dy), ws)
    else:
        call('pidm_conv2d_wgrad_simt', x, dy, gw_buf, gb_buf, B, H, W, Cin, spec.cin_real, Ho, Wo, Cout, KH, KW,
             stride, pad, 1 if spec.transposed else 0, spec.w_stride_n, spec.w_stride_c, _code(x), ws)
    return dx, gw_ret, gb_ret


def conv2d(x, weight, bias, spec, residual=None, gn_link=None, skip=None):
    return _Conv2d.apply(x.contiguous(), weight, bias, None if residual is None else residual.contiguous(), spec,
                         gn_link, skip)


class _GroupNormSilu(torch.autograd.Function):
    @staticmethod
    def forward(ctx, x, gamma, beta, scale_shift, groups, eps, link, residual):
        B, H, W, C = x.shape
        y = torch.empty_like(x)
        pre = link is not None and link.get('sums') is not None
        sums = link['sums'] if pre else torch.empty(B, groups, 2, device=x.device, dtype=torch.float32)
        call('pidm_groupnorm_silu_fwd', x, gamma, beta, scale_shift, residual, y, sums, 1 if pre else 0, B, H * W, C,
             groups, eps, _code(x), stream())
        ctx.save_for_backward(x, gamma, beta, scale_shift, sums)
        ctx.groups, ctx.eps, ctx.link, ctx.has_res = groups, eps, link, residual is not None
        return y

    @staticmethod
    def backward(ctx, dy):
        x, gamma, beta, ss, sums = ctx.saved_tensors
        B, H, W, C = x.shape
        dy = dy.contiguous()
        dx = torch.empty_like(x)
        gg_buf, gg_ret = _grad_buffer(gamma)
        gb_buf, gb_ret = _grad_buffer(beta)
        dss = None if ss is None else torch.empty_like(ss)
        ws = torch.empty(B * C * 2, device=x.device, dtype=torch.float32)
        dbias = None
        link = ctx.link
        if link is not None and link.get('bias') is not None:
            dbias, dbias_ret = _grad_buffer(link['bias'])
            link['dbias'] = dbias_ret
        call('pidm_groupnorm_silu_bwd', x, dy, sums, gamma, beta, ss, dx, gg_buf, gb_buf, dss, dbias, ws, B, H * W, C,
             ctx.groups, ctx.eps, _code(x), stream())
        return dx, gg_ret, gb_ret, dss, None, None, None, (dy if ctx.has_res else None)


def groupnorm_silu(x, gamma, beta, scale_shift, groups, eps=1e-5, gn_link=None, residual=None):
    return _GroupNormSilu.apply(x.contiguous(), gamma, beta, scale_shift, groups, eps, gn_link,
                                None if residual is None else residual.contiguous())


class _LayerNormC(torch.autograd.Function):
    @staticmethod
    def forward(ctx, x, gamma, eps, skip_link):
        C = x.shape[-1]
        y = torch.empty_like(x)
        call('pidm_layernorm_c_fwd', x, gamma, y, x.numel() // C, C, eps, _code(x), stream())
        ctx.save_for_backward(x, gamma)
        ctx.eps, ctx.skip_link = eps, skip_link
        return y

    @staticmethod
    def backward(ctx, dy):
        x, gamma = ctx.saved_tensors
        C = x.shape[-1]
        dy = dy.contiguous()
        dx = torch.empty_like(x)
        gg_buf, gg_ret = _grad_buffer(gamma)
        call('pidm_layernorm_c_bwd', x, dy, gamma, dx, gg_buf,
             _take_skip(ctx.skip_link) if ctx.needs_input_grad[0] else None, x.numel() // C, C, ctx.eps,
             _code(x), stream())
        return dx, gg_ret, None, None


def layernorm_c(x, gamma, eps=1e-5, skip_link=None):
    return _LayerNormC.apply(x.contiguous(), gamma, eps, skip_link)


class _LinAttn(torch.autograd.Function):
    @staticmethod
    def forward(ctx, qkv, heads):
        B, H, W, C3 = qkv.shape
        N = H * W
        hid = heads * 32
        assert C3 == 3 * hid
        out = torch.empty(B, H, W, hid, device=qkv.device, dtype=qkv.dtype)
        ctxm = torch.empty(B, heads, 32, 32, device=qkv.device, dtype=torch.float32)
        kmax = torch.empty(B, heads, 32, device=qkv.device, dtype=torch.float32)
        kzinv = torch.empty_like(kmax)
        ws = torch.empty(call('pidm_linattn_workspace_floats', B, N, heads), device=qkv.device, dtype=torch.float32)
        call('pidm_linattn_fwd', qkv, out, ctxm, kmax, kzinv, ws, B, N, heads, _code(qkv), stream())
        ctx.save_for_backward(qkv, ctxm, kmax, kzinv)
        ctx.heads = heads
        return out

    @staticmethod
    def backward(ctx, dout):
        qkv, ctxm, kmax, kzinv = ctx.saved_tensors
        B, H, W, _ = qkv.shape
        dout = dout.contiguous()
        dqkv = torch.empty_like(qkv)
        dctx = torch.empty_like(ctxm)
        call('pidm_linattn_bwd', qkv, dout, ctxm, kmax, kzinv, dqkv, dctx, B, H * W, ctx.heads, _code(qkv), stream())
        return dqkv, None


class _LinAttnFused(torch.autograd.Function):

    @staticmethod
    def forward(ctx, xn, weight, spec, heads):
        B, H, W, C = xn.shape
        N = H * W
        out = torch.empty(B, H, W, heads * 32, device=xn.device, dtype=xn.dtype)
        ctxm = torch.empty(B, heads, 32, 32, device=xn.device, dtype=torch.float32)
        kmax = torch.empty(B, heads, 32, device=xn.device, dtype=torch.float32)
        kzinv = torch.empty_like(kmax)
        ws = torch.empty(call('pidm_linattn_fused_workspace_floats', B, N), device=xn.device, dtype=torch.float32)
        call('pidm_linattn_fused_fwd', xn, spec.wp_fwd, out, ctxm, kmax, kzinv, ws, B, N, stream())
        ctx.save_for_backward(xn, weight, ctxm, kmax, kzinv)
        ctx.spec, ctx.heads = spec, heads
        return out

    @staticmethod
    def backward(ctx, dout):
        xn, weight, ctxm, kmax, kzinv = ctx.saved_tensors
        spec = ctx.spec
        B, H, W, _ = xn.shape
        dout = dout.contiguous()
        dx = torch.empty_like(xn)
        dctx = torch.empty_like(ctxm)
        call('pidm_linattn_fused_bwd', xn, spec.wp_fwd, dout, ctxm, kmax, kzinv, dx, dctx, B, H * W, stream())
        gw_buf, gw_ret = _grad_buffer(weight)
        ws = _wgrad_stream(xn, spec.wp_fwd, dout, ctxm, dctx, kmax, kzinv)
        call('pidm_linattn_fused_wgrad', xn, spec.wp_fwd, dout, ctxm, dctx, kmax, kzinv, gw_buf, B, H * W,
             spec.w_stride_n, spec.w_stride_c, ws)
        return (dx if ctx.needs_input_grad[0] else None), gw_ret, None, None


def linear_attention_fused_supported(xn, spec, heads):
    B, H, W, C = xn.shape
    return (_STATE['use_tc'] and xn.is_cuda and spec.kh == 1 and spec.kw == 1 and spec.cout == 3 * heads * 32
            and bool(call('pidm_linattn_fused_supported', C, heads, H * W, _code(xn))))


def linear_attention_fused(xn, weight, spec, heads):
    return _LinAttnFused.apply(xn.contiguous(), weight, spec, heads)


def linear_attention(qkv, heads):
    return _LinAttn.apply(qkv.contiguous(), heads)


class _Attn(torch.autograd.Function):
    @staticmethod
    def forward(ctx, qkv, heads):
        B, H, W, C3 = qkv.shape
        out = torch.empty(B, H, W, heads * 32, device=qkv.device, dtype=qkv.dtype)
        call('pidm_attn_fwd', qkv, out, B, H * W, heads, _code(qkv), stream())
        ctx.save_for_backward(qkv)
        ctx.heads = heads
        return out

    @staticmethod
    def backward(ctx, dout):
        (qkv,) = ctx.saved_tensors
        B, H, W, _ = qkv.shape
        dqkv = torch.empty_like(qkv)
        call('pidm_attn_bwd', qkv, dout.contiguous(), dqkv, B, H * W, ctx.heads, _code(qkv), stream())
        return dqkv, None


def softmax_attention(qkv, heads):
    return _Attn.apply(qkv.contiguous(), heads)


class _TimeEmbed(torch.autograd.Function):
    @staticmethod
    def forward(ctx, t, W1, b1, W2, b2):
        B = t.shape[0]
        td, dim = W1.shape
        dev = W1.device
        emb = torch.empty(B, dim, device=dev, dtype=torch.float32)
        h1 = torch.empty(B, td, device=dev, dtype=torch.float32)
        temb = torch.empty_like(h1)
        silu_t = torch.empty_like(h1)
        call('pidm_time_embed_fwd', t, W1, b1, W2, b2, emb, h1, temb, silu_t, B, dim, td, stream())
        ctx.save_for_backward(emb, h1, temb, W1, b1, W2, b2)
        ctx.mark_non_differentiable(temb)
        return silu_t, temb

    @staticmethod
    def backward(ctx, d_silu, _unused):
        emb, h1, temb, W1, b1, W2, b2 = ctx.saved_tensors
        B, td = h1.shape
        gW1, rW1 = _grad_buffer(W1)
        gb1, rb1 = _grad_buffer(b1)
        gW2, rW2 = _grad_buffer(W2)
        gb2, rb2 = _grad_buffer(b2)
        d_silu = d_silu.contiguous()
        ws = torch.empty(2 * B * td, device=h1.device, dtype=torch.float32)
        args = (d_silu, emb, h1, temb, W2, gW1, gb1, gW2, gb2, ws, B, emb.shape[1], td)
        call('pidm_time_embed_bwd', *args, 2, stream())
        call('pidm_time_embed_bwd', *args, 1, _wgrad_stream(ws, emb, h1))
        return None, rW1, rb1, rW2, rb2


def time_embed(t, W1, b1, W2, b2):
    return _TimeEmbed.apply(t.to(torch.int64).contiguous(), W1, b1, W2, b2)


class _BlockMlps(torch.autograd.Function):

    @staticmethod
    def forward(ctx, silu_t, table, *wb):
        B, td = silu_t.shape
        outs = [torch.empty(B, n, device=silu_t.device, dtype=torch.float32) for n in table.rows]
        call('pidm_block_mlps_fwd', table.device_table(outs), table.n, table.max_rows, silu_t, B, td, stream())
        ctx.save_for_backward(silu_t, *wb)
        ctx.table = table
        return tuple(outs)

    @staticmethod
    def backward(ctx, *d_outs):
        silu_t, *wb = ctx.saved_tensors
        table = ctx.table
        B, td = silu_t.shape
        bufs, rets = [], []
        for p in wb:
            b_, r_ = _grad_buffer(p)
            bufs.append(b_)
            rets.append(r_)
        d_outs = [d.contiguous() for d in d_outs]
        d_silu = torch.empty_like(silu_t)
        tab = table.device_table(None, d_outs, bufs)
        call('pidm_block_mlps_bwd', tab, table.n, table.max_rows, silu_t, d_silu, B, td, 1,
             _wgrad_stream(silu_t, tab, *d_outs))
        call('pidm_block_mlps_bwd', tab, table.n, table.max_rows, silu_t, d_silu, B, td, 2, stream())
        return (d_silu, None, *rets)


def block_mlps(silu_t, table):
    return _BlockMlps.apply(silu_t, table, *table.params)


class _Head(torch.autograd.Function):
    @staticmethod
    def forward(ctx, x, w, b, sigmoid_last):
        B, H, W, C = x.shape
        O = w.shape[0]
        y = torch.empty(B, O, H, W, device=x.device, dtype=torch.float32)
        call('pidm_head_fwd', x, w, b, y, B, H * W, C, O, int(sigmoid_last), _code(x), stream())
        ctx.save_for_backward(x, w, b, y)
        ctx.sig = int(sigmoid_last)
        return y

    @staticmethod
    def backward(ctx, dy):
        x, w, b, y = ctx.saved_tensors
        B, H, W, C = x.shape
        O = w.shape[0]
        dx = torch.empty_like(x)
        gw, rw = _grad_buffer(w)
        gb, rb = _grad_buffer(b)
        call('pidm_head_bwd', x, w, y, dy.contiguous().float(), dx, gw, gb, B, H * W, C, O, ctx.sig, _code(x), stream())
        return dx, rw, rb, None


def head(x, w, b, sigmoid_last=False):
    return _Head.apply(x.contiguous(), w, b, sigmoid_last)


def q_sample(x0, noise, t, sqrt_ab, sqrt_1mab):
    _need_cuda(x0, noise, t)
    _need_f32(sqrt_ab=sqrt_ab, sqrt_1mab=sqrt_1mab)
    x0 = x0.contiguous().float()
    xt = torch.empty_like(x0)
    call('pidm_qsample', x0, noise.contiguous().float(), t.to(torch.int64).contiguous(), sqrt_ab, sqrt_1mab, xt,
         x0.shape[0], x0[0].numel(), stream())
    return xt


def posterior_step(x_t, x0_pred, z, c1, c2, sigma):
    out = torch.empty_like(x_t)
    call('pidm_posterior_step', x_t.contiguous(), x0_pred.contiguous(), z.contiguous(), out, float(c1), float(c2),
         float(sigma), x_t.numel(), stream())
    return out


class _DarcyResidual(torch.autograd.Function):
    @staticmethod
    def forward(ctx, x0hat, f_s, geom):
        B, C, P, _ = x0hat.shape
        r = torch.empty(B, P * P, 3, device=x0hat.device, dtype=torch.float32)
        call('pidm_darcy_residual_fwd', x0hat, f_s, r, B, P, *geom, stream())
        ctx.save_for_backward(x0hat, f_s)
        ctx.geom = geom
        return r

    @staticmethod
    def backward(ctx, gr):
        x0hat, f_s = ctx.saved_tensors
        B, C, P, _ = x0hat.shape
        gx = torch.empty_like(x0hat)
        call('pidm_darcy_residual_bwd', x0hat, f_s, gr.contiguous(), gx, B, P, *ctx.geom, stream())
        return gx, None, None


DARCY_PIXELS_AT_BOUNDARY = 1
DARCY_PERIODIC = 2


def darcy_flags(pixels_at_boundary, periodic=False):
    return (DARCY_PIXELS_AT_BOUNDARY if pixels_at_boundary else 0) | (DARCY_PERIODIC if periodic else 0)


def darcy_residual(x0hat, f_s, domain_length=1.0, reverse_d1=True, pixels_at_boundary=True, periodic=False):
    _need_cuda(x0hat)
    _need_f32(f_s=f_s)
    assert x0hat.shape[1] == 2, 'Darcy fields are (p, K)'
    return _DarcyResidual.apply(x0hat.contiguous().float(), f_s,
                                (float(domain_length), int(reverse_d1), darcy_flags(pixels_at_boundary, periodic)))


class _DarcyPidmLoss(torch.autograd.Function):

    @staticmethod
    def forward(ctx, x0hat, model_out, target, t, f_s, p2w, pvar, c_data, c_res, geom):
        B, C, P, _ = x0hat.shape
        same = model_out is None
        sums = torch.empty(3, device=x0hat.device, dtype=torch.float32)
        need = x0hat.requires_grad or (model_out is not None and model_out.requires_grad)
        gx = torch.empty_like(x0hat) if need else None
        gm = None if (same or not need) else torch.empty_like(model_out)
        call('pidm_darcy_pidm_loss', x0hat, x0hat if same else model_out, target, f_s, t, p2w, pvar, float(c_data),
             float(c_res), sums, gx, gm, B, P, *geom, stream())
        ctx.save_for_backward(gx, gm)
        ctx.mark_non_differentiable(sums)
        return sums[0] + sums[1], sums

    @staticmethod
    def backward(ctx, g, _unused):
        gx, gm = ctx.saved_tensors
        g = g.contiguous().float()
        ox = torch.empty_like(gx)
        call('pidm_scale', gx, g, ox, gx.numel(), stream())
        om = None
        if gm is not None:
            om = torch.empty_like(gm)
            call('pidm_scale', gm, g, om, gm.numel(), stream())
        return ox, om, None, None, None, None, None, None, None, None


def darcy_pidm_loss(x0hat, model_out, target, t, f_s, p2w, pvar, c_data, c_res, domain_length=1.0, reverse_d1=True,
                    pixels_at_boundary=True, periodic=False):
    _need_cuda(x0hat, target)
    _need_f32(f_s=f_s, p2w=p2w, pvar=pvar)
    geom = (float(domain_length), int(reverse_d1), darcy_flags(pixels_at_boundary, periodic))
    if model_out is not None and model_out is x0hat:
        model_out = None
    return _DarcyPidmLoss.apply(x0hat.contiguous().float(),
                                None if model_out is None else model_out.contiguous().float(),
                                target.contiguous().float(), t.to(torch.int64).contiguous(), f_s, p2w, pvar, c_data, c_res,
                                geom)
```

Baseline: 6567.

## Extend fused linear attention kernels to 64 input channels

Templates the fused linear-attention forward, backward and weight-gradient kernels on the input channel count so C=64 layers can use them. With C=64 the QKV weights are staged in shared memory instead of registers, and the input tiles are split into two 32-channel chunks. Layers with C=64 and N>=1024 now use the fused path instead of the separate projection plus attention kernels. In exchange the C=64 variant runs with lower occupancy (one block per SM) and uses more shared memory.

```diff
diff --git a/include/pidm.h b/include/pidm.h
--- a/include/pidm.h
+++ b/include/pidm.h
@@ -102,6 +102,16 @@
 int pidm_linattn_fused_wgrad(const void* xn, const void* w_qkv, const void* dout, const float* ctx, const float* dctx,
                              const float* kmax, const float* kzinv, float* grad_w, int B, int N, long long w_stride_n,
                              long long w_stride_c, void* stream);
+int pidm_linattn_fused_c_supported(int C, int heads, int N, int dtype);
+int pidm_linattn_fused_c_workspace_floats(int B, int N, int C);
+int pidm_linattn_fused_c_plan(int B, int N, int C, int* out);
+int pidm_linattn_fused_c_fwd(const void* xn, const void* w_qkv, void* out, float* ctx, float* kmax, float* kzinv,
+                             float* workspace, int B, int N, int C, void* stream);
+int pidm_linattn_fused_c_bwd(const void* xn, const void* w_qkv, const void* dout, const float* ctx, const float* kmax,
+                             const float* kzinv, void* dxn, float* dctx, int B, int N, int C, void* stream);
+int pidm_linattn_fused_c_wgrad(const void* xn, const void* w_qkv, const void* dout, const float* ctx, const float* dctx,
+                               const float* kmax, const float* kzinv, float* grad_w, int B, int N, int C,
+                               long long w_stride_n, long long w_stride_c, void* stream);
 int pidm_linattn_workspace_floats(int B, int N, int heads);
 int pidm_linattn_fwd(const void* qkv, void* out, float* ctx, float* kmax, float* kzinv, float* workspace, int B, int N,
                      int heads, int dtype, void* stream);
diff --git a/physicsinformeddiffusionmodels_b200/_lib.py b/physicsinformeddiffusionmodels_b200/_lib.py
--- a/physicsinformeddiffusionmodels_b200/_lib.py
+++ b/physicsinformeddiffusionmodels_b200/_lib.py
@@ -56,6 +56,12 @@
     'pidm_linattn_fused_fwd': [P, P, P, P, P, P, P, I, I, P],
     'pidm_linattn_fused_bwd': [P, P, P, P, P, P, P, P, I, I, P],
     'pidm_linattn_fused_wgrad': [P, P, P, P, P, P, P, P, I, I, L, L, P],
+    'pidm_linattn_fused_c_supported': [I, I, I, I],
+    'pidm_linattn_fused_c_workspace_floats': [I, I, I],
+    'pidm_linattn_fused_c_plan': [I, I, I, P],
+    'pidm_linattn_fused_c_fwd': [P, P, P, P, P, P, P, I, I, I, P],
+    'pidm_linattn_fused_c_bwd': [P, P, P, P, P, P, P, P, I, I, I, P],
+    'pidm_linattn_fused_c_wgrad': [P, P, P, P, P, P, P, P, I, I, I, L, L, P],
     'pidm_linattn_fwd': [P, P, P, P, P, P, I, I, I, I, P],
     'pidm_linattn_bwd': [P, P, P, P, P, P, P, I, I, I, I, P],
     'pidm_attn_fwd': [P, P, I, I, I, I, P],
@@ -78,6 +84,7 @@
 }
 _VALUE_RETURN = {'pidm_pack_entry_size', 'pidm_pack_pair_entry_size', 'pidm_mlp_entry_size', 'pidm_linattn_workspace_floats', 'pidm_version',
                  'pidm_linattn_fused_supported', 'pidm_linattn_fused_workspace_floats',
+                 'pidm_linattn_fused_c_supported', 'pidm_linattn_fused_c_workspace_floats', 'pidm_linattn_fused_c_plan',
                  'pidm_conv2d_tc_supported', 'pidm_conv2d_wgrad_tc_supported', 'pidm_conv2d_tc_general_supported',
                  'pidm_conv2d_tc_plan', 'pidm_conv2d_wgrad_tc_plan', 'pidm_linattn_fused_plan'}
 
diff --git a/physicsinformeddiffusionmodels_b200/csrc/attention_fused.cu b/physicsinformeddiffusionmodels_b200/csrc/attention_fused.cu
--- a/physicsinformeddiffusionmodels_b200/csrc/attention_fused.cu
+++ b/physicsinformeddiffusionmodels_b200/csrc/attention_fused.cu
@@ -7,6 +7,14 @@
 
 constexpr int LF_C = 32;
 
+template <int C>
+struct LfK {
+    static_assert(C == 32 || C == 64, "fused linear attention: C = 32 or 64");
+    static constexpr int KC = C / 32;
+    static constexpr int WP = C + 8;
+    static constexpr int VSH = C == 32 ? 2 : 3;
+};
+
 __device__ __forceinline__ uint32_t movm_t(uint32_t x) {
     uint32_t y;
     asm volatile("movmatrix.sync.aligned.m8n8.trans.b16 %0, %1;" : "=r"(y) : "r"(x));
@@ -24,23 +32,70 @@
             w[ks][nt][1] = __ldg(row + 4);
         }
 }
-template <int MT>
-__device__ __forceinline__ void load_x_frags(uint32_t (&a)[MT][2][4], const __nv_bfloat16* Xs, int lane) {
+template <int C, bool SMEM = (C > 32)>
+struct LafW {
+    uint32_t f[2][4][2];
+    __device__ __forceinline__ void init(const __nv_bfloat16* __restrict__ Wg, const __nv_bfloat16*, int lane) {
+        load_w_frags(f, Wg, lane);
+    }
+    __device__ __forceinline__ void frags(uint32_t (&w)[1][2][4][2], int) const {
+#pragma unroll
+        for (int ks = 0; ks < 2; ++ks)
+#pragma unroll
+            for (int nt = 0; nt < 4; ++nt) { w[0][ks][nt][0] = f[ks][nt][0]; w[0][ks][nt][1] = f[ks][nt][1]; }
+    }
+};
+template <int C>
+struct LafW<C, true> {
+    const __nv_bfloat16* rows;
+    __device__ __forceinline__ void init(const __nv_bfloat16*, const __nv_bfloat16* Ws, int) { rows = Ws; }
+    __device__ __forceinline__ void frags(uint32_t (&w)[LfK<C>::KC][2][4][2], int lane) const {
+#pragma unroll
+        for (int kc = 0; kc < LfK<C>::KC; ++kc)
+#pragma unroll
+            for (int ks = 0; ks < 2; ++ks)
+#pragma unroll
+                for (int np = 0; np < 2; ++np) {
+                    uint32_t b[4];
+                    frag_b_nrows(b, rows, LfK<C>::WP, np * 16, kc * 32 + ks * 16, lane);
+                    w[kc][ks][2 * np][0] = b[0];
+                    w[kc][ks][2 * np][1] = b[1];
+                    w[kc][ks][2 * np + 1][0] = b[2];
+                    w[kc][ks][2 * np + 1][1] = b[3];
+                }
+    }
+};
+template <int C>
+__device__ __forceinline__ void lf_stage_w(__nv_bfloat16* Ws, const __nv_bfloat16* __restrict__ W, int r0, int nrows) {
+    constexpr int VSH = LfK<C>::VSH, V = 1 << VSH;
+    for (int i = threadIdx.x; i < nrows * V; i += blockDim.x)
+        cp_async16(Ws + (i >> VSH) * LfK<C>::WP + (i & (V - 1)) * 8, W + (size_t)(r0 + (i >> VSH)) * C + (i & (V - 1)) * 8);
+    cp_commit();
+}
+template <int C, int MT>
+__device__ __forceinline__ void load_x_frags(uint32_t (&a)[LfK<C>::KC][MT][2][4], const __nv_bfloat16* Xs, int sub, int lane) {
+#pragma unroll
+    for (int kc = 0; kc < LfK<C>::KC; ++kc)
+#pragma unroll
+        for (int mt = 0; mt < MT; ++mt)
+#pragma unroll
+            for (int ks = 0; ks < 2; ++ks) frag_a_rowmajor(a[kc][mt][ks], Xs + kc * sub, LW_PITCH, mt * 16, ks * 16, lane);
+}
+template <int C, int MT>
+__device__ __forceinline__ void project(float (&c)[MT][4][4], const uint32_t (&a)[LfK<C>::KC][MT][2][4], const LafW<C>& w,
+                                        int lane) {
+    uint32_t wf[LfK<C>::KC][2][4][2];
+    w.frags(wf, lane);
 #pragma unroll
     for (int mt = 0; mt < MT; ++mt)
 #pragma unroll
-        for (int ks = 0; ks < 2; ++ks) frag_a_rowmajor(a[mt][ks], Xs, LW_PITCH, mt * 16, ks * 16, lane);
-}
-template <int MT>
-__device__ __forceinline__ void project(float (&c)[MT][4][4], const uint32_t (&a)[MT][2][4], const uint32_t (&w)[2][4][2]) {
-#pragma unroll
-    for (int mt = 0; mt < MT; ++mt)
-#pragma unroll
         for (int nt = 0; nt < 4; ++nt) {
 #pragma unroll
             for (int i = 0; i < 4; ++i) c[mt][nt][i] = 0.f;
 #pragma unroll
-            for (int ks = 0; ks < 2; ++ks) mma_bf16(c[mt][nt], a[mt][ks], w[ks][nt][0], w[ks][nt][1]);
+            for (int kc = 0; kc < LfK<C>::KC; ++kc)
+#pragma unroll
+                for (int ks = 0; ks < 2; ++ks) mma_bf16(c[mt][nt], a[kc][mt][ks], wf[kc][ks][nt][0], wf[kc][ks][nt][1]);
         }
 }
 __device__ __forceinline__ void frag_softmax(float (&c)[4][4], float mul) {
@@ -81,37 +136,55 @@
 }
 
 constexpr int LFS_STAGES = 2;
+template <int C>
+struct LfsCfg {
+    static constexpr int STAGE_ELEMS = LfK<C>::KC * LW_TILE;
+    static constexpr int W_ROWS = C == 32 ? 0 : LM_HID;
+    static constexpr size_t SMEM = (size_t)LM_HEADS * LFS_STAGES * STAGE_ELEMS * 2 + (size_t)W_ROWS * LfK<C>::WP * 2;
+};
+template <int C>
 __global__ void __launch_bounds__(256) laf_kmax_kernel(const __nv_bfloat16* __restrict__ xn,
                                                        const __nv_bfloat16* __restrict__ W, float* __restrict__ part,
                                                        int N, int rows_per_chunk) {
     pdl_trigger();
     pdl_wait();
     extern __shared__ __align__(16) unsigned char raw[];
+    constexpr int KC = LfK<C>::KC, STAGE_ELEMS = LfsCfg<C>::STAGE_ELEMS;
     const int b = blockIdx.y, chunk = blockIdx.x, lane = threadIdx.x & 31, h = threadIdx.x >> 5;
-    __nv_bfloat16* ring = reinterpret_cast<__nv_bfloat16*>(raw) + (size_t)h * (LFS_STAGES * LW_TILE);
+    __nv_bfloat16* ring = reinterpret_cast<__nv_bfloat16*>(raw) + (size_t)h * (LFS_STAGES * STAGE_ELEMS);
+    __nv_bfloat16* Ws = reinterpret_cast<__nv_bfloat16*>(raw) + (size_t)LM_HEADS * LFS_STAGES * STAGE_ELEMS;
     const int n_begin = chunk * rows_per_chunk, n_end = min(N, n_begin + rows_per_chunk);
     const int n_tiles = (n_end - n_begin) / 32;
-    const __nv_bfloat16* xsrc = xn + ((size_t)b * N + n_begin) * LF_C;
+    const __nv_bfloat16* xsrc = xn + ((size_t)b * N + n_begin) * C;
+    if constexpr (C > 32) lf_stage_w<C>(Ws, W, LM_HID, LM_HID);
     auto issue = [&](int it) {
-        if (it < n_tiles) lw_issue<32>(ring + (size_t)(it % LFS_STAGES) * LW_TILE, xsrc + (size_t)it * 32 * LF_C, LF_C, lane);
+        if (it < n_tiles)
+#pragma unroll
+            for (int kc = 0; kc < KC; ++kc)
+                lw_issue<32>(ring + (size_t)(it % LFS_STAGES) * STAGE_ELEMS + kc * LW_TILE, xsrc + (size_t)it * 32 * C + kc * 32,
+                             C, lane);
         cp_commit();
     };
 #pragma unroll
     for (int s = 0; s < LFS_STAGES; ++s) issue(s);
-    uint32_t wk[2][4][2];
-    load_w_frags(wk, W + (size_t)(LM_HID + h * LM_D) * LF_C, lane);
+    if constexpr (C > 32) {
+        cp_wait<LFS_STAGES>();
+        __syncthreads();
+    }
+    LafW<C> wk;
+    wk.init(W + (size_t)(LM_HID + h * LM_D) * C, Ws + (size_t)h * LM_D * LfK<C>::WP, lane);
     float m[8];
 #pragma unroll
     for (int i = 0; i < 8; ++i) m[i] = -INFINITY;
     for (int it = 0; it < n_tiles; ++it) {
         cp_wait<LFS_STAGES - 1>();
         __syncwarp();
-        uint32_t ax[2][2][4];
-        load_x_frags<2>(ax, ring + (size_t)(it % LFS_STAGES) * LW_TILE, lane);
+        uint32_t ax[KC][2][2][4];
+        load_x_frags<C, 2>(ax, ring + (size_t)(it % LFS_STAGES) * STAGE_ELEMS, LW_TILE, lane);
         __syncwarp();
         issue(it + LFS_STAGES);
         float ck[2][4][4];
-        project<2>(ck, ax, wk);
+        project<C, 2>(ck, ax, wk, lane);
 #pragma unroll
         for (int nt = 0; nt < 4; ++nt)
 #pragma unroll
@@ -143,43 +216,53 @@
     if (lane == 0) kzinv[row] = zi;
 }
 
-template <int MODE>
+template <int C, int MODE>
 struct LfcCfg {
-    static constexpr int STAGES = MODE == 0 ? 4 : 2;
-    static constexpr int STAGE_ELEMS = MODE == 0 ? LW_TILE : 2 * LW_TILE;
-    static constexpr size_t SMEM = (size_t)LM_HEADS * STAGES * STAGE_ELEMS * 2 + (size_t)LM_HEADS * 2 * LM_D * 4;
+    static constexpr int STAGES = (MODE == 0 && C == 32) ? 4 : 2;
+    static constexpr int STAGE_ELEMS = (LfK<C>::KC + MODE) * LW_TILE;
+    static constexpr int W_ROWS = C == 32 ? 0 : (MODE == 0 ? 2 : 1) * LM_HID;
+    static constexpr size_t SMEM = (size_t)LM_HEADS * STAGES * STAGE_ELEMS * 2 + (size_t)LM_HEADS * 2 * LM_D * 4 +
+                                   (size_t)W_ROWS * LfK<C>::WP * 2;
 };
-template <int MODE>
-__global__ void __launch_bounds__(256, 2) laf_ctx_kernel(const __nv_bfloat16* __restrict__ xn, const __nv_bfloat16* __restrict__ W,
+template <int C, int MODE>
+__global__ void __launch_bounds__(256, C == 32 ? 2 : 1) laf_ctx_kernel(const __nv_bfloat16* __restrict__ xn, const __nv_bfloat16* __restrict__ W,
                                                       const __nv_bfloat16* __restrict__ dout, const float* __restrict__ part,
                                                       int n_stat_chunks, float* __restrict__ kmax, float* __restrict__ kzinv,
                                                       float* __restrict__ ctx, int N, int chunk_px, float scale) {
     pdl_trigger();
     pdl_wait();
     extern __shared__ __align__(16) unsigned char raw[];
-    constexpr int LFC_STAGES = LfcCfg<MODE>::STAGES, LFC_STAGE_ELEMS = LfcCfg<MODE>::STAGE_ELEMS;
+    constexpr int KC = LfK<C>::KC, WP = LfK<C>::WP;
+    constexpr int LFC_STAGES = LfcCfg<C, MODE>::STAGES, LFC_STAGE_ELEMS = LfcCfg<C, MODE>::STAGE_ELEMS;
     const int b = blockIdx.y, chunk = blockIdx.x, lane = threadIdx.x & 31, h = threadIdx.x >> 5;
     __nv_bfloat16* ring = reinterpret_cast<__nv_bfloat16*>(raw) + (size_t)h * (LFC_STAGES * LFC_STAGE_ELEMS);
     float* sM = reinterpret_cast<float*>(raw + (size_t)LM_HEADS * LFC_STAGES * LFC_STAGE_ELEMS * 2) + h * 2 * LM_D;
-    float* sZi = sM + LM_D;
+    __nv_bfloat16* Ws = reinterpret_cast<__nv_bfloat16*>(raw + (size_t)LM_HEADS * LFC_STAGES * LFC_STAGE_ELEMS * 2 +
+                                                         (size_t)LM_HEADS * 2 * LM_D * 4);
     const int n_begin = chunk * chunk_px, n_end = min(N, n_begin + chunk_px);
     const int n_tiles = (n_end - n_begin) / 32;
     const size_t pix0 = (size_t)b * N + n_begin;
-    const __nv_bfloat16* xsrc = xn + pix0 * LF_C;
+    const __nv_bfloat16* xsrc = xn + pix0 * C;
     const __nv_bfloat16* gsrc = (MODE == 1) ? dout + pix0 * LM_HID + h * LM_D : nullptr;
+    if constexpr (C > 32) lf_stage_w<C>(Ws, W, MODE == 0 ? LM_HID : 0, LfcCfg<C, MODE>::W_ROWS);
     auto issue = [&](int it) {
         if (it < n_tiles) {
             __nv_bfloat16* buf = ring + (size_t)(it % LFC_STAGES) * LFC_STAGE_ELEMS;
-            lw_issue<32>(buf, xsrc + (size_t)it * 32 * LF_C, LF_C, lane);
-            if (MODE == 1) lw_issue<32>(buf + LW_TILE, gsrc + (size_t)it * 32 * LM_HID, LM_HID, lane);
+#pragma unroll
+            for (int kc = 0; kc < KC; ++kc) lw_issue<32>(buf + kc * LW_TILE, xsrc + (size_t)it * 32 * C + kc * 32, C, lane);
+            if (MODE == 1) lw_issue<32>(buf + KC * LW_TILE, gsrc + (size_t)it * 32 * LM_HID, LM_HID, lane);
         }
         cp_commit();
     };
 #pragma unroll
     for (int s = 0; s < LFC_STAGES; ++s) issue(s);
-    uint32_t w0[2][4][2], w1[2][4][2];
-    load_w_frags(w0, W + (size_t)((MODE == 0 ? LM_HID : 0) + h * LM_D) * LF_C, lane);
-    if (MODE == 0) load_w_frags(w1, W + (size_t)(2 * LM_HID + h * LM_D) * LF_C, lane);
+    if constexpr (C > 32) {
+        cp_wait<LFC_STAGES>();
+        __syncthreads();
+    }
+    LafW<C> w0, w1;
+    w0.init(W + (size_t)((MODE == 0 ? LM_HID : 0) + h * LM_D) * C, Ws + (size_t)h * LM_D * WP, lane);
+    if (MODE == 0) w1.init(W + (size_t)(2 * LM_HID + h * LM_D) * C, Ws + (size_t)(LM_HID + h * LM_D) * WP, lane);
     float Mc[8];
     float zacc[8];
 #pragma unroll
@@ -204,15 +287,15 @@
         cp_wait<LFC_STAGES - 1>();
         __syncwarp();
         const __nv_bfloat16* buf = ring + (size_t)(it % LFC_STAGES) * LFC_STAGE_ELEMS;
-        uint32_t ax[2][2][4];
-        load_x_frags<2>(ax, buf, lane);
+        uint32_t ax[KC][2][2][4];
+        load_x_frags<C, 2>(ax, buf, LW_TILE, lane);
         uint32_t bv[2][4][2];
         if (MODE == 1) {
 #pragma unroll
             for (int ks = 0; ks < 2; ++ks) {
                 uint32_t b01[4], b23[4];
-                frag_b_krows(b01, buf + LW_TILE, LW_PITCH, ks * 16, 0, lane);
-                frag_b_krows(b23, buf + LW_TILE, LW_PITCH, ks * 16, 16, lane);
+                frag_b_krows(b01, buf + KC * LW_TILE, LW_PITCH, ks * 16, 0, lane);
+                frag_b_krows(b23, buf + KC * LW_TILE, LW_PITCH, ks * 16, 16, lane);
                 bv[ks][0][0] = b01[0]; bv[ks][0][1] = b01[1]; bv[ks][1][0] = b01[2]; bv[ks][1][1] = b01[3];
                 bv[ks][2][0] = b23[0]; bv[ks][2][1] = b23[1]; bv[ks][3][0] = b23[2]; bv[ks][3][1] = b23[3];
             }
@@ -220,7 +303,7 @@
         __syncwarp();
         issue(it + LFC_STAGES);
         float cw[2][4][4];
-        project<2>(cw, ax, w0);
+        project<C, 2>(cw, ax, w0, lane);
         if (MODE == 0) {
 #pragma unroll
             for (int mt = 0; mt < 2; ++mt)
@@ -232,7 +315,7 @@
                         zacc[nt * 2 + (i & 1)] += cw[mt][nt][i];
                     }
             float cv[2][4][4];
-            project<2>(cv, ax, w1);
+            project<C, 2>(cv, ax, w1, lane);
 #pragma unroll
             for (int mt = 0; mt < 2; ++mt)
 #pragma unroll
@@ -289,28 +372,45 @@
 }
 
 constexpr int LFO_STAGES = 2;
+template <int C>
+struct LfoCfg {
+    static constexpr int WARP_ELEMS = (LFO_STAGES * LfK<C>::KC + 1) * LW_TILE;
+    static constexpr int W_ROWS = C == 32 ? 0 : LM_HID;
+    static constexpr size_t SMEM = (size_t)LM_HEADS * WARP_ELEMS * 2 + (size_t)W_ROWS * LfK<C>::WP * 2;
+};
+template <int C>
 __global__ void __launch_bounds__(256) laf_out_kernel(const __nv_bfloat16* __restrict__ xn, const __nv_bfloat16* __restrict__ W,
                                                       const float* __restrict__ ctx, __nv_bfloat16* __restrict__ out, int N,
                                                       int chunk_px, float scale) {
     pdl_trigger();
     pdl_wait();
     extern __shared__ __align__(16) unsigned char raw[];
+    constexpr int KC = LfK<C>::KC;
     const int b = blockIdx.y, chunk = blockIdx.x, lane = threadIdx.x & 31, h = threadIdx.x >> 5;
-    __nv_bfloat16* ring = reinterpret_cast<__nv_bfloat16*>(raw) + (size_t)h * ((LFO_STAGES + 1) * LW_TILE);
-    __nv_bfloat16* Os = ring + LFO_STAGES * LW_TILE;
+    __nv_bfloat16* ring = reinterpret_cast<__nv_bfloat16*>(raw) + (size_t)h * LfoCfg<C>::WARP_ELEMS;
+    __nv_bfloat16* Os = ring + LFO_STAGES * KC * LW_TILE;
+    __nv_bfloat16* Ws = reinterpret_cast<__nv_bfloat16*>(raw) + (size_t)LM_HEADS * LfoCfg<C>::WARP_ELEMS;
     const int n_begin = chunk * chunk_px, n_end = min(N, n_begin + chunk_px);
     const int n_tiles = (n_end - n_begin) / 32;
     const size_t pix0 = (size_t)b * N + n_begin;
-    const __nv_bfloat16* xsrc = xn + pix0 * LF_C;
+    const __nv_bfloat16* xsrc = xn + pix0 * C;
     __nv_bfloat16* odst = out + pix0 * LM_HID + h * LM_D;
+    if constexpr (C > 32) lf_stage_w<C>(Ws, W, 0, LM_HID);
     auto issue = [&](int it) {
-        if (it < n_tiles) lw_issue<32>(ring + (size_t)(it % LFO_STAGES) * LW_TILE, xsrc + (size_t)it * 32 * LF_C, LF_C, lane);
+        if (it < n_tiles)
+#pragma unroll
+            for (int kc = 0; kc < KC; ++kc)
+                lw_issue<32>(ring + (size_t)((it % LFO_STAGES) * KC + kc) * LW_TILE, xsrc + (size_t)it * 32 * C + kc * 32, C, lane);
         cp_commit();
     };
 #pragma unroll
     for (int s = 0; s < LFO_STAGES; ++s) issue(s);
-    uint32_t wq[2][4][2];
-    load_w_frags(wq, W + (size_t)(h * LM_D) * LF_C, lane);
+    if constexpr (C > 32) {
+        cp_wait<LFO_STAGES>();
+        __syncthreads();
+    }
+    LafW<C> wq;
+    wq.init(W + (size_t)(h * LM_D) * C, Ws + (size_t)h * LM_D * LfK<C>::WP, lane);
     const float* ch = ctx + ((size_t)b * LM_HEADS + h) * LM_D * LM_D;
     uint32_t bf[2][4][2];
 #pragma unroll
@@ -321,12 +421,12 @@
     for (int it = 0; it < n_tiles; ++it) {
         cp_wait<LFO_STAGES - 1>();
         __syncwarp();
-        uint32_t ax[2][2][4];
-        load_x_frags<2>(ax, ring + (size_t)(it % LFO_STAGES) * LW_TILE, lane);
+        uint32_t ax[KC][2][2][4];
+        load_x_frags<C, 2>(ax, ring + (size_t)(it % LFO_STAGES) * KC * LW_TILE, LW_TILE, lane);
         __syncwarp();
         issue(it + LFO_STAGES);
         float cq[2][4][4];
-        project<2>(cq, ax, wq);
+        project<C, 2>(cq, ax, wq, lane);
 #pragma unroll
         for (int mt = 0; mt < 2; ++mt) {
             frag_softmax(cq[mt], scale);
@@ -358,13 +458,15 @@
 constexpr int LFB_STAGES = 4;
 constexpr int LFB_TILE = LFB_ROWS * LW_PITCH;
 
+template <int C>
 struct LfbTile {
-    uint32_t ax[1][2][4], ag[2][4];
+    uint32_t ax[LfK<C>::KC][1][2][4], ag[2][4];
 };
-__device__ __forceinline__ void lfb_dq(float (&dq)[4][4], const LfbTile& tl, const uint32_t (&wq)[2][4][2],
-                                       const uint32_t (&bc)[2][4][2], float scale) {
+template <int C>
+__device__ __forceinline__ void lfb_dq(float (&dq)[4][4], const LfbTile<C>& tl, const LafW<C>& wq,
+                                       const uint32_t (&bc)[2][4][2], float scale, int lane) {
     float c1[1][4][4], c2[4][4];
-    project<1>(c1, tl.ax, wq);
+    project<C, 1>(c1, tl.ax, wq, lane);
     frag_softmax(c1[0], 1.f);
 #pragma unroll
     for (int nt = 0; nt < 4; ++nt) {
@@ -387,29 +489,34 @@
             for (int j = 0; j < 2; ++j) dq[nt][half * 2 + j] = scale * c1[0][nt][half * 2 + j] * (c2[nt][half * 2 + j] - dot);
     }
 }
-__device__ __forceinline__ void lfb_dkdv(float (&dk)[4][4], float (&dv)[4][4], const uint32_t (&ax)[1][2][4],
-                                         const uint32_t (&wk)[2][4][2], const uint32_t (&wv)[2][4][2],
+template <int C, bool DK = true, bool DV = true>
+__device__ __forceinline__ void lfb_dkdv(float (&dk)[4][4], float (&dv)[4][4], const uint32_t (&ax)[LfK<C>::KC][1][2][4],
+                                         const LafW<C>& wk, const LafW<C>& wv,
                                          const uint32_t (&bd)[2][4][2], const uint32_t (&bt)[2][4][2],
-                                         const float (&Mc)[8], const float (&Zc)[8], const float (&cdc)[8], float invN) {
+                                         const float (&Mc)[8], const float (&Zc)[8], const float (&cdc)[8], float invN,
+                                         int lane) {
     float c1[1][4][4];
     uint32_t a[2][4];
-    project<1>(c1, ax, wv);
-    c_to_a(a, c1[0]);
-#pragma unroll
-    for (int nt = 0; nt < 4; ++nt) {
-#pragma unroll
-        for (int i = 0; i < 4; ++i) dk[nt][i] = 0.f;
-#pragma unroll
-        for (int ks = 0; ks < 2; ++ks) mma_bf16(dk[nt], a[ks], bd[ks][nt][0], bd[ks][nt][1]);
-    }
-    project<1>(c1, ax, wk);
+    if (DK) {
+        project<C, 1>(c1, ax, wv, lane);
+        c_to_a(a, c1[0]);
+#pragma unroll
+        for (int nt = 0; nt < 4; ++nt) {
+#pragma unroll
+            for (int i = 0; i < 4; ++i) dk[nt][i] = 0.f;
+#pragma unroll
+            for (int ks = 0; ks < 2; ++ks) mma_bf16(dk[nt], a[ks], bd[ks][nt][0], bd[ks][nt][1]);
+        }
+    }
+    project<C, 1>(c1, ax, wk, lane);
 #pragma unroll
     for (int nt = 0; nt < 4; ++nt)
 #pragma unroll
         for (int i = 0; i < 4; ++i) {
             c1[0][nt][i] = __expf(c1[0][nt][i] - Mc[nt * 2 + (i & 1)]) * Zc[nt * 2 + (i & 1)];
-            dk[nt][i] = c1[0][nt][i] * (dk[nt][i] * invN - cdc[nt * 2 + (i & 1)]);
-        }
+            if (DK) dk[nt][i] = c1[0][nt][i] * (dk[nt][i] * invN - cdc[nt * 2 + (i & 1)]);
+        }
+    if (!DV) return;
     c_to_a(a, c1[0]);
 #pragma unroll
     for (int nt = 0; nt < 4; ++nt) {
@@ -435,24 +542,29 @@
     load_cols(cdc, scd, lane);
 }
 
-constexpr int LFB_STAGE_ELEMS = (1 + LM_HEADS) * LFB_TILE;
-constexpr int LFB_W_PITCH = LF_C + 8;
-constexpr int LFB_R_PITCH = LF_C + 8;
-constexpr size_t LAF_BWD_SMEM = (size_t)LFB_STAGES * LFB_STAGE_ELEMS * 2 + (size_t)3 * LM_HID * LFB_W_PITCH * 2 +
-                                (size_t)LM_HEADS * LFB_ROWS * LFB_R_PITCH * 4 + (size_t)LM_HEADS * LM_D * 4;
-
-__device__ __forceinline__ void mma_w(float (&c)[4][4], const uint32_t (&g)[2][4], const __nv_bfloat16* Wh, int lane) {
+template <int C>
+struct LfbCfg {
+    static constexpr int STAGE_ELEMS = (LfK<C>::KC + LM_HEADS) * LFB_TILE;
+    static constexpr int W_PITCH = LfK<C>::WP;
+    static constexpr int R_PITCH = C + 8;
+    static constexpr size_t SMEM = (size_t)LFB_STAGES * STAGE_ELEMS * 2 + (size_t)3 * LM_HID * W_PITCH * 2 +
+                                   (size_t)LM_HEADS * LFB_ROWS * R_PITCH * 4 + (size_t)LM_HEADS * LM_D * 4;
+};
+
+template <int C>
+__device__ __forceinline__ void mma_w(float (&c)[C / 8][4], const uint32_t (&g)[2][4], const __nv_bfloat16* Wh, int lane) {
 #pragma unroll
     for (int kd = 0; kd < 2; ++kd)
 #pragma unroll
-        for (int np = 0; np < 2; ++np) {
+        for (int np = 0; np < C / 16; ++np) {
             uint32_t bw[4];
-            frag_b_krows(bw, Wh, LFB_W_PITCH, kd * 16, np * 16, lane);
+            frag_b_krows(bw, Wh, LfK<C>::WP, kd * 16, np * 16, lane);
             mma_bf16(c[2 * np], g[kd], bw[0], bw[1]);
             mma_bf16(c[2 * np + 1], g[kd], bw[2], bw[3]);
         }
 }
 
+template <int C>
 __global__ void __launch_bounds__(256) laf_bwd_kernel(const __nv_bfloat16* __restrict__ xn, const __nv_bfloat16* __restrict__ W,
                                                       const __nv_bfloat16* __restrict__ dout, const float* __restrict__ ctx,
                                                       const float* __restrict__ dctx, const float* __restrict__ kmax,
@@ -461,24 +573,27 @@
     pdl_trigger();
     pdl_wait();
     extern __shared__ __align__(16) unsigned char raw[];
+    constexpr int KC = LfK<C>::KC, STAGE_ELEMS = LfbCfg<C>::STAGE_ELEMS, W_PITCH = LfbCfg<C>::W_PITCH,
+                  R_PITCH = LfbCfg<C>::R_PITCH;
     const int b = blockIdx.y, chunk = blockIdx.x, lane = threadIdx.x & 31, h = threadIdx.x >> 5;
     __nv_bfloat16* ring = reinterpret_cast<__nv_bfloat16*>(raw);
-    __nv_bfloat16* Ws = ring + LFB_STAGES * LFB_STAGE_ELEMS;
-    float* R = reinterpret_cast<float*>(Ws + 3 * LM_HID * LFB_W_PITCH);
-    float* scd = R + LM_HEADS * LFB_ROWS * LFB_R_PITCH + h * LM_D;
+    __nv_bfloat16* Ws = ring + LFB_STAGES * STAGE_ELEMS;
+    float* R = reinterpret_cast<float*>(Ws + 3 * LM_HID * W_PITCH);
+    float* scd = R + LM_HEADS * LFB_ROWS * R_PITCH + h * LM_D;
     const int n_begin = chunk * chunk_px, n_end = min(N, n_begin + chunk_px);
     const int n_tiles = (n_end - n_begin) / LFB_ROWS;
     const size_t pix0 = (size_t)b * N + n_begin;
-    const __nv_bfloat16* xsrc = xn + pix0 * LF_C;
+    const __nv_bfloat16* xsrc = xn + pix0 * C;
     const __nv_bfloat16* gsrc = dout + pix0 * LM_HID + h * LM_D;
-    for (int i = threadIdx.x; i < 3 * LM_HID * (LF_C / 8); i += blockDim.x)
-        cp_async16(Ws + (i >> 2) * LFB_W_PITCH + (i & 3) * 8, W + (size_t)(i >> 2) * LF_C + (i & 3) * 8);
-    cp_commit();
+    lf_stage_w<C>(Ws, W, 0, 3 * LM_HID);
     auto issue = [&](int it) {
         if (it < n_tiles) {
-            __nv_bfloat16* buf = ring + (size_t)(it % LFB_STAGES) * LFB_STAGE_ELEMS;
-            if (h == 0) lw_issue<LFB_ROWS>(buf, xsrc + (size_t)it * LFB_ROWS * LF_C, LF_C, lane);
-            lw_issue<LFB_ROWS>(buf + (1 + h) * LFB_TILE, gsrc + (size_t)it * LFB_ROWS * LM_HID, LM_HID, lane);
+            __nv_bfloat16* buf = ring + (size_t)(it % LFB_STAGES) * STAGE_ELEMS;
+            if (h == 0)
+#pragma unroll
+                for (int kc = 0; kc < KC; ++kc)
+                    lw_issue<LFB_ROWS>(buf + kc * LFB_TILE, xsrc + (size_t)it * LFB_ROWS * C + kc * 32, C, lane);
+            lw_issue<LFB_ROWS>(buf + (KC + h) * LFB_TILE, gsrc + (size_t)it * LFB_ROWS * LM_HID, LM_HID, lane);
         }
         cp_commit();
     };
@@ -490,10 +605,13 @@
     lfb_cd(cdc, scd, cg, dg, lane);
     load_cols(Mc, kmax + (size_t)b * LM_HID + h * LM_D, lane);
     load_cols(Zc, kzinv + (size_t)b * LM_HID + h * LM_D, lane);
-    uint32_t wq[2][4][2], wk[2][4][2], wv[2][4][2];
-    load_w_frags(wq, W + (size_t)(h * LM_D) * LF_C, lane);
-    load_w_frags(wk, W + (size_t)(LM_HID + h * LM_D) * LF_C, lane);
-    load_w_frags(wv, W + (size_t)(2 * LM_HID + h * LM_D) * LF_C, lane);
+    const __nv_bfloat16* Wq = Ws + (size_t)(h * LM_D) * W_PITCH;
+    const __nv_bfloat16* Wk = Wq + (size_t)LM_HID * W_PITCH;
+    const __nv_bfloat16* Wv = Wk + (size_t)LM_HID * W_PITCH;
+    LafW<C> wq, wk, wv;
+    wq.init(W + (size_t)(h * LM_D) * C, Wq, lane);
+    wk.init(W + (size_t)(LM_HID + h * LM_D) * C, Wk, lane);
+    wv.init(W + (size_t)(2 * LM_HID + h * LM_D) * C, Wv, lane);
     uint32_t bc[2][4][2], bd[2][4][2], bt[2][4][2];
 #pragma unroll
     for (int ks = 0; ks < 2; ++ks)
@@ -505,68 +623,71 @@
         }
     const int g = lane >> 2, t = lane & 3;
     const float invN = 1.f / (float)N;
-    const __nv_bfloat16* Wq = Ws + (size_t)(h * LM_D) * LFB_W_PITCH;
-    const __nv_bfloat16* Wk = Wq + (size_t)LM_HID * LFB_W_PITCH;
-    const __nv_bfloat16* Wv = Wk + (size_t)LM_HID * LFB_W_PITCH;
-    float* Rw = R + h * LFB_ROWS * LFB_R_PITCH;
+    float* Rw = R + h * LFB_ROWS * R_PITCH;
     const int rrow = threadIdx.x >> 4, rcol = (threadIdx.x & 15) * 2;
     for (int it = 0; it < n_tiles; ++it) {
         cp_wait<LFB_STAGES - 2>();
         __syncthreads();
         issue(it + LFB_STAGES - 1);
-        const __nv_bfloat16* buf = ring + (size_t)(it % LFB_STAGES) * LFB_STAGE_ELEMS;
-        LfbTile tl;
-        load_x_frags<1>(tl.ax, buf, lane);
-        frag_a_rowmajor(tl.ag[0], buf + (1 + h) * LFB_TILE, LW_PITCH, 0, 0, lane);
-        frag_a_rowmajor(tl.ag[1], buf + (1 + h) * LFB_TILE, LW_PITCH, 0, 16, lane);
-        float dx[4][4];
-#pragma unroll
-        for (int nt = 0; nt < 4; ++nt)
+        const __nv_bfloat16* buf = ring + (size_t)(it % LFB_STAGES) * STAGE_ELEMS;
+        LfbTile<C> tl;
+        load_x_frags<C, 1>(tl.ax, buf, LFB_TILE, lane);
+        frag_a_rowmajor(tl.ag[0], buf + (KC + h) * LFB_TILE, LW_PITCH, 0, 0, lane);
+        frag_a_rowmajor(tl.ag[1], buf + (KC + h) * LFB_TILE, LW_PITCH, 0, 16, lane);
+        float dx[C / 8][4];
+#pragma unroll
+        for (int nt = 0; nt < C / 8; ++nt)
 #pragma unroll
             for (int i = 0; i < 4; ++i) dx[nt][i] = 0.f;
         uint32_t a[2][4];
         {
             float dq[4][4];
-            lfb_dq(dq, tl, wq, bc, scale);
+            lfb_dq<C>(dq, tl, wq, bc, scale, lane);
             c_to_a(a, dq);
-            mma_w(dx, a, Wq, lane);
+            mma_w<C>(dx, a, Wq, lane);
         }
         {
             float dk[4][4], dv[4][4];
-            lfb_dkdv(dk, dv, tl.ax, wk, wv, bd, bt, Mc, Zc, cdc, invN);
+            lfb_dkdv<C>(dk, dv, tl.ax, wk, wv, bd, bt, Mc, Zc, cdc, invN, lane);
             c_to_a(a, dk);
-            mma_w(dx, a, Wk, lane);
+            mma_w<C>(dx, a, Wk, lane);
             c_to_a(a, dv);
-            mma_w(dx, a, Wv, lane);
-        }
-#pragma unroll
-        for (int nt = 0; nt < 4; ++nt)
+            mma_w<C>(dx, a, Wv, lane);
+        }
+#pragma unroll
+        for (int nt = 0; nt < C / 8; ++nt)
 #pragma unroll
             for (int half = 0; half < 2; ++half)
-                *reinterpret_cast<float2*>(Rw + (g + half * 8) * LFB_R_PITCH + nt * 8 + 2 * t) =
+                *reinterpret_cast<float2*>(Rw + (g + half * 8) * R_PITCH + nt * 8 + 2 * t) =
                     make_float2(dx[nt][half * 2], dx[nt][half * 2 + 1]);
         __syncthreads();
-        float sx = 0.f, sy = 0.f;
-#pragma unroll
-        for (int w = 0; w < LM_HEADS; ++w) {
-            const float2 v = *reinterpret_cast<const float2*>(R + (w * LFB_ROWS + rrow) * LFB_R_PITCH + rcol);
-            sx += v.x;
-            sy += v.y;
-        }
-        *reinterpret_cast<uint32_t*>(dxn + (pix0 + (size_t)it * LFB_ROWS + rrow) * LF_C + rcol) = pack_bf16(sx, sy);
-    }
-}
-
-template <int PART>
+#pragma unroll
+        for (int kc = 0; kc < KC; ++kc) {
+            float sx = 0.f, sy = 0.f;
+#pragma unroll
+            for (int w = 0; w < LM_HEADS; ++w) {
+                const float2 v = *reinterpret_cast<const float2*>(R + (w * LFB_ROWS + rrow) * R_PITCH + kc * 32 + rcol);
+                sx += v.x;
+                sy += v.y;
+            }
+            *reinterpret_cast<uint32_t*>(dxn + (pix0 + (size_t)it * LFB_ROWS + rrow) * C + kc * 32 + rcol) = pack_bf16(sx, sy);
+        }
+    }
+}
+
+template <int C, int PART>
 struct LfwCfg {
-    static constexpr int MATS = PART == 0 ? 1 : 2;
-    static constexpr int STAGE_ELEMS = (PART == 0 ? 2 : 1) * LFB_TILE;
-    static constexpr int S_PITCH = LM_D + 1;
+    static constexpr int MATS = (C == 32 && PART == 1) ? 2 : 1;
+    static constexpr bool DV = PART == 2 || (C == 32 && PART == 1);
+    static constexpr int STAGE_ELEMS = (LfK<C>::KC + (PART == 0 ? 1 : 0)) * LFB_TILE;
+    static constexpr int S_PITCH = C + 1;
     static_assert(LFB_STAGES * STAGE_ELEMS * 2 >= LM_D * S_PITCH * 4, "the epilogue staging reuses the tile ring");
-    static constexpr size_t SMEM = (size_t)LM_HEADS * (LFB_STAGES * STAGE_ELEMS * 2 + LM_D * 4);
+    static constexpr int W_R0 = PART == 0 ? 0 : LM_HID, W_ROWS = C == 32 ? 0 : (PART == 1 ? 2 : 1) * LM_HID;
+    static constexpr size_t SMEM = (size_t)LM_HEADS * (LFB_STAGES * STAGE_ELEMS * 2 + LM_D * 4) + (size_t)W_ROWS * LfK<C>::WP * 2;
 };
 
-__device__ __forceinline__ void acc_gtx(float (&acc)[2][4][4], const float (&gf)[4][4], const uint32_t (&bx)[2][4]) {
+template <int C>
+__device__ __forceinline__ void acc_gtx(float (&acc)[2][C / 8][4], const float (&gf)[4][4], const uint32_t (&bx)[C / 16][4]) {
 #pragma unroll
     for (int md = 0; md < 2; ++md) {
         uint32_t a[4];
@@ -575,14 +696,14 @@
         a[2] = movm_t(pack_bf16(gf[2 * md][2], gf[2 * md][3]));
         a[3] = movm_t(pack_bf16(gf[2 * md + 1][2], gf[2 * md + 1][3]));
 #pragma unroll
-        for (int np = 0; np < 2; ++np) {
+        for (int np = 0; np < C / 16; ++np) {
             mma_bf16(acc[md][2 * np], a, bx[np][0], bx[np][1]);
             mma_bf16(acc[md][2 * np + 1], a, bx[np][2], bx[np][3]);
         }
     }
 }
 
-template <int PART>
+template <int C, int PART>
 __global__ void __launch_bounds__(256) laf_wgrad_kernel(const __nv_bfloat16* __restrict__ xn, const __nv_bfloat16* __restrict__ W,
                                                         const __nv_bfloat16* __restrict__ dout, const float* __restrict__ ctx,
                                                         const float* __restrict__ dctx, const float* __restrict__ kmax,
@@ -591,80 +712,93 @@
     pdl_trigger();
     pdl_wait();
     extern __shared__ __align__(16) unsigned char raw[];
-    constexpr int MATS = LfwCfg<PART>::MATS, STAGE_ELEMS = LfwCfg<PART>::STAGE_ELEMS, S_PITCH = LfwCfg<PART>::S_PITCH;
+    constexpr int KC = LfK<C>::KC, WP = LfK<C>::WP;
+    constexpr int MATS = LfwCfg<C, PART>::MATS, STAGE_ELEMS = LfwCfg<C, PART>::STAGE_ELEMS, S_PITCH = LfwCfg<C, PART>::S_PITCH;
+    constexpr bool DV = LfwCfg<C, PART>::DV;
     const int b = blockIdx.y, chunk = blockIdx.x, lane = threadIdx.x & 31, h = threadIdx.x >> 5;
     __nv_bfloat16* ring = reinterpret_cast<__nv_bfloat16*>(raw) + (size_t)h * (LFB_STAGES * STAGE_ELEMS);
     float* scd = reinterpret_cast<float*>(raw + (size_t)LM_HEADS * LFB_STAGES * STAGE_ELEMS * 2) + h * LM_D;
+    __nv_bfloat16* Ws = reinterpret_cast<__nv_bfloat16*>(raw + (size_t)LM_HEADS * (LFB_STAGES * STAGE_ELEMS * 2 + LM_D * 4));
     const int n_begin = chunk * chunk_px, n_end = min(N, n_begin + chunk_px);
     const int n_tiles = (n_end - n_begin) / LFB_ROWS;
     const size_t pix0 = (size_t)b * N + n_begin;
-    const __nv_bfloat16* xsrc = xn + pix0 * LF_C;
+    const __nv_bfloat16* xsrc = xn + pix0 * C;
     const __nv_bfloat16* gsrc = dout + pix0 * LM_HID + h * LM_D;
+    if constexpr (C > 32) lf_stage_w<C>(Ws, W, LfwCfg<C, PART>::W_R0, LfwCfg<C, PART>::W_ROWS);
     auto issue = [&](int it) {
         if (it < n_tiles) {
             __nv_bfloat16* buf = ring + (size_t)(it % LFB_STAGES) * STAGE_ELEMS;
-            lw_issue<LFB_ROWS>(buf, xsrc + (size_t)it * LFB_ROWS * LF_C, LF_C, lane);
-            if (PART == 0) lw_issue<LFB_ROWS>(buf + LFB_TILE, gsrc + (size_t)it * LFB_ROWS * LM_HID, LM_HID, lane);
+#pragma unroll
+            for (int kc = 0; kc < KC; ++kc)
+                lw_issue<LFB_ROWS>(buf + kc * LFB_TILE, xsrc + (size_t)it * LFB_ROWS * C + kc * 32, C, lane);
+            if (PART == 0) lw_issue<LFB_ROWS>(buf + KC * LFB_TILE, gsrc + (size_t)it * LFB_ROWS * LM_HID, LM_HID, lane);
         }
         cp_commit();
     };
 #pragma unroll
     for (int s = 0; s < LFB_STAGES; ++s) issue(s);
+    if constexpr (C > 32) {
+        cp_wait<LFB_STAGES>();
+        __syncthreads();
+    }
     const float* cg = ctx + ((size_t)b * LM_HEADS + h) * LM_D * LM_D;
     const float* dg = dctx + ((size_t)b * LM_HEADS + h) * LM_D * LM_D;
     float Mc[8], Zc[8], cdc[8];
-    uint32_t w0[2][4][2], w1[2][4][2];
+    LafW<C> w0, w1;
     uint32_t b0[2][4][2], b1[2][4][2];
     if (PART == 0) {
-        load_w_frags(w0, W + (size_t)(h * LM_D) * LF_C, lane);
+        w0.init(W + (size_t)(h * LM_D) * C, Ws + (size_t)h * LM_D * WP, lane);
     } else {
         lfb_cd(cdc, scd, cg, dg, lane);
         load_cols(Mc, kmax + (size_t)b * LM_HID + h * LM_D, lane);
         load_cols(Zc, kzinv + (size_t)b * LM_HID + h * LM_D, lane);
-        load_w_frags(w0, W + (size_t)(LM_HID + h * LM_D) * LF_C, lane);
-        load_w_frags(w1, W + (size_t)(2 * LM_HID + h * LM_D) * LF_C, lane);
+        w0.init(W + (size_t)(LM_HID + h * LM_D) * C, Ws + (size_t)h * LM_D * WP, lane);
+        if (PART == 1) w1.init(W + (size_t)(2 * LM_HID + h * LM_D) * C, Ws + (size_t)(LM_HID + h * LM_D) * WP, lane);
     }
 #pragma unroll
     for (int ks = 0; ks < 2; ++ks)
 #pragma unroll
         for (int nt = 0; nt < 4; ++nt) {
-            frag_b_global<false>(b0[ks][nt], PART == 0 ? cg : dg, ks * 16, nt * 8, lane);
-            if (PART == 1) frag_b_global<true>(b1[ks][nt], dg, ks * 16, nt * 8, lane);
+            if (PART < 2) frag_b_global<false>(b0[ks][nt], PART == 0 ? cg : dg, ks * 16, nt * 8, lane);
+            if (DV) frag_b_global<true>(b1[ks][nt], dg, ks * 16, nt * 8, lane);
         }
     const float invN = 1.f / (float)N;
-    float acc[MATS][2][4][4];
+    float acc[MATS][2][C / 8][4];
 #pragma unroll
     for (int m = 0; m < MATS; ++m)
 #pragma unroll
         for (int i = 0; i < 2; ++i)
 #pragma unroll
-            for (int j = 0; j < 4; ++j)
+            for (int j = 0; j < C / 8; ++j)
 #pragma unroll
                 for (int k = 0; k < 4; ++k) acc[m][i][j][k] = 0.f;
     for (int it = 0; it < n_tiles; ++it) {
         cp_wait<LFB_STAGES - 1>();
         __syncwarp();
         const __nv_bfloat16* buf = ring + (size_t)(it % LFB_STAGES) * STAGE_ELEMS;
-        LfbTile tl;
-        load_x_frags<1>(tl.ax, buf, lane);
-        uint32_t bx[2][4];
-        frag_b_krows(bx[0], buf, LW_PITCH, 0, 0, lane);
-        frag_b_krows(bx[1], buf, LW_PITCH, 0, 16, lane);
+        LfbTile<C> tl;
+        load_x_frags<C, 1>(tl.ax, buf, LFB_TILE, lane);
+        uint32_t bx[C / 16][4];
+#pragma unroll
+        for (int kc = 0; kc < KC; ++kc) {
+            frag_b_krows(bx[2 * kc], buf + kc * LFB_TILE, LW_PITCH, 0, 0, lane);
+            frag_b_krows(bx[2 * kc + 1], buf + kc * LFB_TILE, LW_PITCH, 0, 16, lane);
+        }
         if (PART == 0) {
-            frag_a_rowmajor(tl.ag[0], buf + LFB_TILE, LW_PITCH, 0, 0, lane);
-            frag_a_rowmajor(tl.ag[1], buf + LFB_TILE, LW_PITCH, 0, 16, lane);
+            frag_a_rowmajor(tl.ag[0], buf + KC * LFB_TILE, LW_PITCH, 0, 0, lane);
+            frag_a_rowmajor(tl.ag[1], buf + KC * LFB_TILE, LW_PITCH, 0, 16, lane);
         }
         __syncwarp();
         issue(it + LFB_STAGES);
         if (PART == 0) {
             float dq[4][4];
-            lfb_dq(dq, tl, w0, b0, scale);
-            acc_gtx(acc[0], dq, bx);
+            lfb_dq<C>(dq, tl, w0, b0, scale, lane);
+            acc_gtx<C>(acc[0], dq, bx);
         } else {
             float dk[4][4], dv[4][4];
-            lfb_dkdv(dk, dv, tl.ax, w0, w1, b0, b1, Mc, Zc, cdc, invN);
-            acc_gtx(acc[0], dk, bx);
-            acc_gtx(acc[MATS - 1], dv, bx);
+            lfb_dkdv<C, PART == 1, DV>(dk, dv, tl.ax, w0, w1, b0, b1, Mc, Zc, cdc, invN, lane);
+            if (PART == 1) acc_gtx<C>(acc[0], dk, bx);
+            if (DV) acc_gtx<C>(acc[MATS - 1], dv, bx);
         }
     }
     cp_wait<0>();
@@ -676,30 +810,33 @@
 #pragma unroll
         for (int md = 0; md < 2; ++md)
 #pragma unroll
-            for (int nc = 0; nc < 4; ++nc)
+            for (int nc = 0; nc < C / 8; ++nc)
 #pragma unroll
                 for (int i = 0; i < 4; ++i) S[(md * 16 + g + 8 * (i >> 1)) * S_PITCH + nc * 8 + 2 * t + (i & 1)] = acc[m][md][nc][i];
         __syncwarp();
         float* dst = grad_w + (long long)((PART + m) * LM_HID + h * LM_D) * w_stride_n + lane * w_stride_c;
+#pragma unroll
+        for (int kc = 0; kc < KC; ++kc)
 #pragma unroll 4
-        for (int d = 0; d < LM_D; ++d) atomicAdd(dst + d * w_stride_n, S[d * S_PITCH + lane]);
-        __syncwarp();
-    }
-}
-
-constexpr size_t LAF_STATS_SMEM = (size_t)LM_HEADS * LFS_STAGES * LW_TILE * 2;
-constexpr size_t LAF_OUT_SMEM = (size_t)LM_HEADS * (LFO_STAGES + 1) * LW_TILE * 2;
-
+            for (int d = 0; d < LM_D; ++d) atomicAdd(dst + kc * 32 * w_stride_c + d * w_stride_n, S[d * S_PITCH + kc * 32 + lane]);
+        __syncwarp();
+    }
+}
+
+template <int C>
 static int laf_attrs() {
     static bool done = false;
     if (!done) {
-        PIDM_CUDA(cudaFuncSetAttribute(laf_kmax_kernel, cudaFuncAttributeMaxDynamicSharedMemorySize, (int)LAF_STATS_SMEM));
-        PIDM_CUDA(cudaFuncSetAttribute(laf_ctx_kernel<0>, cudaFuncAttributeMaxDynamicSharedMemorySize, (int)LfcCfg<0>::SMEM));
-        PIDM_CUDA(cudaFuncSetAttribute(laf_ctx_kernel<1>, cudaFuncAttributeMaxDynamicSharedMemorySize, (int)LfcCfg<1>::SMEM));
-        PIDM_CUDA(cudaFuncSetAttribute(laf_out_kernel, cudaFuncAttributeMaxDynamicSharedMemorySize, (int)LAF_OUT_SMEM));
-        PIDM_CUDA(cudaFuncSetAttribute(laf_bwd_kernel, cudaFuncAttributeMaxDynamicSharedMemorySize, (int)LAF_BWD_SMEM));
-        PIDM_CUDA(cudaFuncSetAttribute(laf_wgrad_kernel<0>, cudaFuncAttributeMaxDynamicSharedMemorySize, (int)LfwCfg<0>::SMEM));
-        PIDM_CUDA(cudaFuncSetAttribute(laf_wgrad_kernel<1>, cudaFuncAttributeMaxDynamicSharedMemorySize, (int)LfwCfg<1>::SMEM));
+        PIDM_CUDA(cudaFuncSetAttribute(laf_kmax_kernel<C>, cudaFuncAttributeMaxDynamicSharedMemorySize, (int)LfsCfg<C>::SMEM));
+        PIDM_CUDA(cudaFuncSetAttribute(laf_ctx_kernel<C, 0>, cudaFuncAttributeMaxDynamicSharedMemorySize, (int)LfcCfg<C, 0>::SMEM));
+        PIDM_CUDA(cudaFuncSetAttribute(laf_ctx_kernel<C, 1>, cudaFuncAttributeMaxDynamicSharedMemorySize, (int)LfcCfg<C, 1>::SMEM));
+        PIDM_CUDA(cudaFuncSetAttribute(laf_out_kernel<C>, cudaFuncAttributeMaxDynamicSharedMemorySize, (int)LfoCfg<C>::SMEM));
+        PIDM_CUDA(cudaFuncSetAttribute(laf_bwd_kernel<C>, cudaFuncAttributeMaxDynamicSharedMemorySize, (int)LfbCfg<C>::SMEM));
+        PIDM_CUDA(cudaFuncSetAttribute(laf_wgrad_kernel<C, 0>, cudaFuncAttributeMaxDynamicSharedMemorySize, (int)LfwCfg<C, 0>::SMEM));
+        PIDM_CUDA(cudaFuncSetAttribute(laf_wgrad_kernel<C, 1>, cudaFuncAttributeMaxDynamicSharedMemorySize, (int)LfwCfg<C, 1>::SMEM));
+        if constexpr (C > 32)
+            PIDM_CUDA(cudaFuncSetAttribute(laf_wgrad_kernel<C, 2>, cudaFuncAttributeMaxDynamicSharedMemorySize,
+                                           (int)LfwCfg<C, 2>::SMEM));
         done = true;
     }
     return 0;
@@ -720,6 +857,90 @@
     return c;
 }
 
+template <int C>
+static void laf_ctas_per_sm(int (&v)[4]) {
+    const int c32[4] = {2, 3, 1, 1}, wide[4] = {1, 1, 1, 1};
+    for (int i = 0; i < 4; ++i) v[i] = C == 32 ? c32[i] : wide[i];
+}
+
+template <int C>
+static void laf_plan(int B, int N, int (&v)[5]) {
+    int cps[4];
+    laf_ctas_per_sm<C>(cps);
+    v[0] = laf_stat_chunks(N);
+    for (int i = 0; i < 4; ++i) v[1 + i] = laf_chunk_px(B, N, cps[i]);
+}
+
+template <int C>
+static int laf_fwd(const void* xn, const void* w_qkv, void* out, float* ctx, float* kmax, float* kzinv, float* workspace,
+                   int B, int N, cudaStream_t st) {
+    if (int e = laf_attrs<C>()) return e;
+    const float scale = 0.17677669529663687f;
+    const __nv_bfloat16* x = (const __nv_bfloat16*)xn;
+    const __nv_bfloat16* w = (const __nv_bfloat16*)w_qkv;
+    int plan[5];
+    laf_plan<C>(B, N, plan);
+    PIDM_CUDA(cudaMemsetAsync(ctx, 0, (size_t)B * LM_HEADS * LM_D * LM_D * sizeof(float), st));
+    PIDM_CUDA(cudaMemsetAsync(kzinv, 0, (size_t)B * LM_HID * sizeof(float), st));
+    const int chunks = plan[0];
+    const int rpc = N / chunks;
+    PIDM_REQUIRE(rpc % 32 == 0 && rpc * chunks == N, "linattn_fused: bad statistics chunking for N=%d", N);
+    PIDM_CUDA(launch_pdl(laf_kmax_kernel<C>, dim3(chunks, B), dim3(256), LfsCfg<C>::SMEM, st, x, w, workspace, N, rpc));
+    const int cpx = plan[1];
+    PIDM_CUDA(launch_pdl(laf_ctx_kernel<C, 0>, dim3((N + cpx - 1) / cpx, B), dim3(256), LfcCfg<C, 0>::SMEM, st, x, w, nullptr,
+                         workspace, chunks, kmax, kzinv, ctx, N, cpx, scale));
+    PIDM_CUDA(launch_pdl(laf_finalize_kernel, dim3((B * LM_HID + 7) / 8), dim3(256), (size_t)(0), st, ctx, kzinv, B * LM_HID));
+    const int opx = plan[2];
+    PIDM_CUDA(launch_pdl(laf_out_kernel<C>, dim3((N + opx - 1) / opx, B), dim3(256), LfoCfg<C>::SMEM, st, x, w, ctx,
+                         (__nv_bfloat16*)out, N, opx, scale));
+    PIDM_LAUNCH_CHECK("linattn_fused_fwd");
+    return 0;
+}
+
+template <int C>
+static int laf_bwd(const void* xn, const void* w_qkv, const void* dout, const float* ctx, const float* kmax,
+                   const float* kzinv, void* dxn, float* dctx, int B, int N, cudaStream_t st) {
+    if (int e = laf_attrs<C>()) return e;
+    const float scale = 0.17677669529663687f;
+    const __nv_bfloat16* x = (const __nv_bfloat16*)xn;
+    const __nv_bfloat16* w = (const __nv_bfloat16*)w_qkv;
+    int plan[5];
+    laf_plan<C>(B, N, plan);
+    PIDM_CUDA(cudaMemsetAsync(dctx, 0, (size_t)B * LM_HEADS * LM_D * LM_D * sizeof(float), st));
+    const int cpx = plan[1];
+    PIDM_CUDA(launch_pdl(laf_ctx_kernel<C, 1>, dim3((N + cpx - 1) / cpx, B), dim3(256), LfcCfg<C, 1>::SMEM, st, x, w,
+                         (const __nv_bfloat16*)dout, nullptr, 0, nullptr, nullptr, dctx, N, cpx, scale));
+    const int bpx = plan[3];
+    PIDM_CUDA(launch_pdl(laf_bwd_kernel<C>, dim3((N + bpx - 1) / bpx, B), dim3(256), LfbCfg<C>::SMEM, st, x, w,
+                         (const __nv_bfloat16*)dout, ctx, dctx, kmax, kzinv, (__nv_bfloat16*)dxn, N, bpx, scale));
+    PIDM_LAUNCH_CHECK("linattn_fused_bwd");
+    return 0;
+}
+
+template <int C>
+static int laf_wgrad(const void* xn, const void* w_qkv, const void* dout, const float* ctx, const float* dctx,
+                     const float* kmax, const float* kzinv, float* grad_w, int B, int N, long long w_stride_n,
+                     long long w_stride_c, cudaStream_t st) {
+    if (int e = laf_attrs<C>()) return e;
+    const float scale = 0.17677669529663687f;
+    const __nv_bfloat16* x = (const __nv_bfloat16*)xn;
+    const __nv_bfloat16* w = (const __nv_bfloat16*)w_qkv;
+    const __nv_bfloat16* g = (const __nv_bfloat16*)dout;
+    int plan[5];
+    laf_plan<C>(B, N, plan);
+    const int px = plan[4];
+    const dim3 grid((N + px - 1) / px, B);
+    PIDM_CUDA(launch_pdl(laf_wgrad_kernel<C, 0>, grid, dim3(256), LfwCfg<C, 0>::SMEM, st, x, w, g, ctx, dctx, kmax, kzinv,
+                         grad_w, N, px, w_stride_n, w_stride_c, scale));
+    PIDM_CUDA(launch_pdl(laf_wgrad_kernel<C, 1>, grid, dim3(256), LfwCfg<C, 1>::SMEM, st, x, w, g, ctx, dctx, kmax, kzinv,
+                         grad_w, N, px, w_stride_n, w_stride_c, scale));
+    if constexpr (C > 32)
+        PIDM_CUDA(launch_pdl(laf_wgrad_kernel<C, 2>, grid, dim3(256), LfwCfg<C, 2>::SMEM, st, x, w, g, ctx, dctx, kmax,
+                             kzinv, grad_w, N, px, w_stride_n, w_stride_c, scale));
+    PIDM_LAUNCH_CHECK("linattn_fused_wgrad");
+    return 0;
+}
+
 }
 using namespace pidm;
 
@@ -731,8 +952,8 @@
 
 extern "C" int pidm_linattn_fused_plan(int B, int N, int* out) {
     PIDM_REQUIRE(N % 128 == 0 && B > 0, "linattn_fused_plan: N must be a multiple of 128 (got %d)", N);
-    const int v[5] = {laf_stat_chunks(N), laf_chunk_px(B, N, 2), laf_chunk_px(B, N, 3), laf_chunk_px(B, N, 1),
-                      laf_chunk_px(B, N, 1)};
+    int v[5];
+    laf_plan<LF_C>(B, N, v);
     for (int i = 0; i < 5; ++i) out[i] = v[i];
     return 0;
 }
@@ -740,63 +961,60 @@
 extern "C" int pidm_linattn_fused_fwd(const void* xn, const void* w_qkv, void* out, float* ctx, float* kmax, float* kzinv,
                                       float* workspace, int B, int N, void* stream) {
     PIDM_REQUIRE(N % 128 == 0, "linattn_fused: N must be a multiple of 128 (got %d)", N);
-    cudaStream_t st = (cudaStream_t)stream;
-    if (int e = laf_attrs()) return e;
-    const float scale = 0.17677669529663687f;
-    const __nv_bfloat16* x = (const __nv_bfloat16*)xn;
-    const __nv_bfloat16* w = (const __nv_bfloat16*)w_qkv;
-    PIDM_CUDA(cudaMemsetAsync(ctx, 0, (size_t)B * LM_HEADS * LM_D * LM_D * sizeof(float), st));
-    PIDM_CUDA(cudaMemsetAsync(kzinv, 0, (size_t)B * LM_HID * sizeof(float), st));
-    const int chunks = laf_stat_chunks(N);
-    const int rpc = N / chunks;
-    PIDM_REQUIRE(rpc % 32 == 0 && rpc * chunks == N, "linattn_fused: bad statistics chunking for N=%d", N);
-    PIDM_CUDA(launch_pdl(laf_kmax_kernel, dim3(dim3(chunks, B)), dim3(256), (size_t)(LAF_STATS_SMEM), st, x, w, workspace, N, rpc));
-    const int cpx = laf_chunk_px(B, N, 2);
-    PIDM_CUDA(launch_pdl(laf_ctx_kernel<0>, dim3(dim3((N + cpx - 1) / cpx, B)), dim3(256), (size_t)(LfcCfg<0>::SMEM), st, x, w, nullptr, workspace, chunks, kmax, kzinv,
-                                                                             ctx, N, cpx, scale));
-    PIDM_CUDA(launch_pdl(laf_finalize_kernel, dim3((B * LM_HID + 7) / 8), dim3(256), (size_t)(0), st, ctx, kzinv, B * LM_HID));
-    const int opx = laf_chunk_px(B, N, 3);
-    PIDM_CUDA(launch_pdl(laf_out_kernel, dim3(dim3((N + opx - 1) / opx, B)), dim3(256), (size_t)(LAF_OUT_SMEM), st, x, w, ctx, (__nv_bfloat16*)out, N, opx, scale));
-    PIDM_LAUNCH_CHECK("linattn_fused_fwd");
-    return 0;
+    return laf_fwd<LF_C>(xn, w_qkv, out, ctx, kmax, kzinv, workspace, B, N, (cudaStream_t)stream);
 }
 
 extern "C" int pidm_linattn_fused_bwd(const void* xn, const void* w_qkv, const void* dout, const float* ctx,
                                       const float* kmax, const float* kzinv, void* dxn, float* dctx, int B, int N,
                                       void* stream) {
     PIDM_REQUIRE(N % 128 == 0, "linattn_fused: N must be a multiple of 128 (got %d)", N);
-    cudaStream_t st = (cudaStream_t)stream;
-    if (int e = laf_attrs()) return e;
-    const float scale = 0.17677669529663687f;
-    const __nv_bfloat16* x = (const __nv_bfloat16*)xn;
-    const __nv_bfloat16* w = (const __nv_bfloat16*)w_qkv;
-    PIDM_CUDA(cudaMemsetAsync(dctx, 0, (size_t)B * LM_HEADS * LM_D * LM_D * sizeof(float), st));
-    const int cpx = laf_chunk_px(B, N, 2);
-    PIDM_CUDA(launch_pdl(laf_ctx_kernel<1>, dim3(dim3((N + cpx - 1) / cpx, B)), dim3(256), (size_t)(LfcCfg<1>::SMEM), st, x, w, (const __nv_bfloat16*)dout, nullptr, 0,
-                                                                             nullptr, nullptr, dctx, N, cpx, scale));
-    const int bpx = laf_chunk_px(B, N, 1);
-    PIDM_CUDA(launch_pdl(laf_bwd_kernel, dim3(dim3((N + bpx - 1) / bpx, B)), dim3(256), (size_t)(LAF_BWD_SMEM), st, x, w, (const __nv_bfloat16*)dout, ctx, dctx, kmax,
-                                                                          kzinv, (__nv_bfloat16*)dxn, N, bpx, scale));
-    PIDM_LAUNCH_CHECK("linattn_fused_bwd");
-    return 0;
+    return laf_bwd<LF_C>(xn, w_qkv, dout, ctx, kmax, kzinv, dxn, dctx, B, N, (cudaStream_t)stream);
 }
 
 extern "C" int pidm_linattn_fused_wgrad(const void* xn, const void* w_qkv, const void* dout, const float* ctx,
                                         const float* dctx, const float* kmax, const float* kzinv, float* grad_w, int B,
                                         int N, long long w_stride_n, long long w_stride_c, void* stream) {
     PIDM_REQUIRE(N % 128 == 0, "linattn_fused: N must be a multiple of 128 (got %d)", N);
-    cudaStream_t st = (cudaStream_t)stream;
-    if (int e = laf_attrs()) return e;
-    const float scale = 0.17677669529663687f;
-    const __nv_bfloat16* x = (const __nv_bfloat16*)xn;
-    const __nv_bfloat16* w = (const __nv_bfloat16*)w_qkv;
-    const __nv_bfloat16* g = (const __nv_bfloat16*)dout;
-    const int px = laf_chunk_px(B, N, 1);
-    const dim3 grid((N + px - 1) / px, B);
-    PIDM_CUDA(launch_pdl(laf_wgrad_kernel<0>, grid, dim3(256), LfwCfg<0>::SMEM, st, x, w, g, ctx, dctx, kmax, kzinv, grad_w, N,
-                         px, w_stride_n, w_stride_c, scale));
-    PIDM_CUDA(launch_pdl(laf_wgrad_kernel<1>, grid, dim3(256), LfwCfg<1>::SMEM, st, x, w, g, ctx, dctx, kmax, kzinv, grad_w, N,
-                         px, w_stride_n, w_stride_c, scale));
-    PIDM_LAUNCH_CHECK("linattn_fused_wgrad");
+    return laf_wgrad<LF_C>(xn, w_qkv, dout, ctx, dctx, kmax, kzinv, grad_w, B, N, w_stride_n, w_stride_c,
+                           (cudaStream_t)stream);
+}
+
+constexpr int LAF_C_MIN_N = 1024;
+static bool laf_c_ok(int C, int N) { return C == 64 && N % 128 == 0; }
+
+extern "C" int pidm_linattn_fused_c_supported(int C, int heads, int N, int dtype) {
+    return (laf_c_ok(C, N) && heads == LM_HEADS && dtype == PIDM_BF16 && N >= LAF_C_MIN_N) ? 1 : 0;
+}
+
+extern "C" int pidm_linattn_fused_c_workspace_floats(int B, int N, int C) {
+    return laf_c_ok(C, N) ? B * laf_stat_chunks(N) * LM_HID : -1;
+}
+
+extern "C" int pidm_linattn_fused_c_plan(int B, int N, int C, int* out) {
+    PIDM_REQUIRE(laf_c_ok(C, N) && B > 0, "linattn_fused_c_plan: C = 64 and N %% 128 == 0 required (got C=%d, N=%d)", C, N);
+    int v[5];
+    laf_plan<64>(B, N, v);
+    for (int i = 0; i < 5; ++i) out[i] = v[i];
     return 0;
 }
+
+extern "C" int pidm_linattn_fused_c_fwd(const void* xn, const void* w_qkv, void* out, float* ctx, float* kmax, float* kzinv,
+                                        float* workspace, int B, int N, int C, void* stream) {
+    PIDM_REQUIRE(laf_c_ok(C, N), "linattn_fused_c: C = 64 and N %% 128 == 0 required (got C=%d, N=%d)", C, N);
+    return laf_fwd<64>(xn, w_qkv, out, ctx, kmax, kzinv, workspace, B, N, (cudaStream_t)stream);
+}
+
+extern "C" int pidm_linattn_fused_c_bwd(const void* xn, const void* w_qkv, const void* dout, const float* ctx,
+                                        const float* kmax, const float* kzinv, void* dxn, float* dctx, int B, int N, int C,
+                                        void* stream) {
+    PIDM_REQUIRE(laf_c_ok(C, N), "linattn_fused_c: C = 64 and N %% 128 == 0 required (got C=%d, N=%d)", C, N);
+    return laf_bwd<64>(xn, w_qkv, dout, ctx, kmax, kzinv, dxn, dctx, B, N, (cudaStream_t)stream);
+}
+
+extern "C" int pidm_linattn_fused_c_wgrad(const void* xn, const void* w_qkv, const void* dout, const float* ctx,
+                                          const float* dctx, const float* kmax, const float* kzinv, float* grad_w, int B,
+                                          int N, int C, long long w_stride_n, long long w_stride_c, void* stream) {
+    PIDM_REQUIRE(laf_c_ok(C, N), "linattn_fused_c: C = 64 and N %% 128 == 0 required (got C=%d, N=%d)", C, N);
+    return laf_wgrad<64>(xn, w_qkv, dout, ctx, dctx, kmax, kzinv, grad_w, B, N, w_stride_n, w_stride_c,
+                         (cudaStream_t)stream);
+}
diff --git a/physicsinformeddiffusionmodels_b200/ops.py b/physicsinformeddiffusionmodels_b200/ops.py
--- a/physicsinformeddiffusionmodels_b200/ops.py
+++ b/physicsinformeddiffusionmodels_b200/ops.py
@@ -416,8 +416,13 @@
         ctxm = torch.empty(B, heads, 32, 32, device=xn.device, dtype=torch.float32)
         kmax = torch.empty(B, heads, 32, device=xn.device, dtype=torch.float32)
         kzinv = torch.empty_like(kmax)
-        ws = torch.empty(call('pidm_linattn_fused_workspace_floats', B, N), device=xn.device, dtype=torch.float32)
-        call('pidm_linattn_fused_fwd', xn, spec.wp_fwd, out, ctxm, kmax, kzinv, ws, B, N, stream())
+        if C == 32:
+            ws = torch.empty(call('pidm_linattn_fused_workspace_floats', B, N), device=xn.device, dtype=torch.float32)
+            call('pidm_linattn_fused_fwd', xn, spec.wp_fwd, out, ctxm, kmax, kzinv, ws, B, N, stream())
+        else:
+            ws = torch.empty(call('pidm_linattn_fused_c_workspace_floats', B, N, C), device=xn.device,
+                             dtype=torch.float32)
+            call('pidm_linattn_fused_c_fwd', xn, spec.wp_fwd, out, ctxm, kmax, kzinv, ws, B, N, C, stream())
         ctx.save_for_backward(xn, weight, ctxm, kmax, kzinv)
         ctx.spec, ctx.heads = spec, heads
         return out
@@ -426,22 +431,31 @@
     def backward(ctx, dout):
         xn, weight, ctxm, kmax, kzinv = ctx.saved_tensors
         spec = ctx.spec
-        B, H, W, _ = xn.shape
+        B, H, W, C = xn.shape
         dout = dout.contiguous()
         dx = torch.empty_like(xn)
         dctx = torch.empty_like(ctxm)
-        call('pidm_linattn_fused_bwd', xn, spec.wp_fwd, dout, ctxm, kmax, kzinv, dx, dctx, B, H * W, stream())
+        if C == 32:
+            call('pidm_linattn_fused_bwd', xn, spec.wp_fwd, dout, ctxm, kmax, kzinv, dx, dctx, B, H * W, stream())
+        else:
+            call('pidm_linattn_fused_c_bwd', xn, spec.wp_fwd, dout, ctxm, kmax, kzinv, dx, dctx, B, H * W, C, stream())
         gw_buf, gw_ret = _grad_buffer(weight)
         ws = _wgrad_stream(xn, spec.wp_fwd, dout, ctxm, dctx, kmax, kzinv)
-        call('pidm_linattn_fused_wgrad', xn, spec.wp_fwd, dout, ctxm, dctx, kmax, kzinv, gw_buf, B, H * W,
-             spec.w_stride_n, spec.w_stride_c, ws)
+        if C == 32:
+            call('pidm_linattn_fused_wgrad', xn, spec.wp_fwd, dout, ctxm, dctx, kmax, kzinv, gw_buf, B, H * W,
+                 spec.w_stride_n, spec.w_stride_c, ws)
+        else:
+            call('pidm_linattn_fused_c_wgrad', xn, spec.wp_fwd, dout, ctxm, dctx, kmax, kzinv, gw_buf, B, H * W, C,
+                 spec.w_stride_n, spec.w_stride_c, ws)
         return (dx if ctx.needs_input_grad[0] else None), gw_ret, None, None
 
 
 def linear_attention_fused_supported(xn, spec, heads):
     B, H, W, C = xn.shape
-    return (_STATE['use_tc'] and xn.is_cuda and spec.kh == 1 and spec.kw == 1 and spec.cout == 3 * heads * 32
-            and bool(call('pidm_linattn_fused_supported', C, heads, H * W, _code(xn))))
+    return (_STATE['use_tc'] and xn.is_cuda and spec.kh == 1 and spec.kw == 1 and spec.cin == C
+            and spec.cout == 3 * heads * 32
+            and (bool(call('pidm_linattn_fused_supported', C, heads, H * W, _code(xn)))
+                 or bool(call('pidm_linattn_fused_c_supported', C, heads, H * W, _code(xn)))))
 
 
 def linear_attention_fused(xn, weight, spec, heads):
```

Result: no change. 6589, median of 6 (+0.3%).
